# ShreenathKR2000/DFU-Multimodal

Hardware: AMD Instinct MI355X
Metric: images/sec (fusion fwd+bwd, bs=64/GPU) (higher is better)
Workload: dtype fwd ResNet50 bf16x3, ViT-B/16 Blocks fp16 (fp32 accumulate, residual stream, statistics); bwd bf16 MFMA; fp32 master weights / AdamW

## Files before the change

### dfu-multimodal_amd/csrc/gemm.hip

```cpp
#include <math.h>
#include <stdlib.h>

#include <type_traits>

#include "gemm_table.h"

using namespace dfu;

namespace {

inline int round8(int x) { return (x + 7) & ~7; }
inline int cdiv(int a, int b) { return (a + b - 1) / b; }

constexpr int kCUs = 256;
struct TileInfo {
  int tm, tn, occ;
  bool phased, tail_ok;
  double step_us, round_us;
  const Entry* kernels;
  const int* nkernels;
  int slots() const { return kCUs * occ; }
  int tiles(int M, int N) const { return cdiv(M, tm) * cdiv(N, tn); }
};
#define X(name, tm, tn, occ, phased, tail_ok, step_us, round_us) \
// ... 297 lines not shown
      DFU_CHECK_ARG(d->conv_k % BK == 0, "dfu_gemm: conv dgrad needs Kout %% 64 == 0");
      DFU_CHECK_ARG(d->K == d->conv_r * d->conv_s * d->conv_k, "dfu_gemm: conv dgrad K != RSK");
      DFU_CHECK_ARG(d->M == d->conv_n * d->conv_h * d->conv_w, "dfu_gemm: conv dgrad M != NHW");
      DFU_CHECK_ARG(d->conv_c % 8 == 0, "dfu_gemm: conv dgrad needs C %% 8 == 0");
      DFU_CHECK_ARG(d->b_mode == DFU_OPND_CONV_DGRAD_W, "dfu_gemm: conv dgrad needs DGRAD_W B");
    }
    if (d->b_mode == DFU_OPND_CONV_WGRAD_X) {
      DFU_CHECK_ARG(d->conv_c % 8 == 0, "dfu_gemm: conv wgrad needs C %% 8 == 0");
      DFU_CHECK_ARG(d->N == d->conv_r * d->conv_s * d->conv_c, "dfu_gemm: conv wgrad N != RSC");
      DFU_CHECK_ARG(d->K == d->conv_n * d->conv_p * d->conv_q, "dfu_gemm: conv wgrad K != NPQ");
    }
  }
  return DFU_OK;
}

}

extern "C" int dfu_gemm_stats_tiles(int32_t M) { return (M + 127) / 128; }

extern "C" int64_t dfu_gemm_workspace_bytes(const dfu_gemm_desc* d) {
  if (!d) return 0;
  const Plan pl = plan_gemm(d);
  if (!pl.entry) return 0;
  if (d->epilogue != DFU_EPI_F32_ACC) {
    if (!g_tail_split) return 0;
    if (d->a_mode == DFU_OPND_CONV_DGRAD && d->conv_stride > 1) {
      int64_t b = 0;
      for (const TileInfo& ti : kTiles) {
        const int64_t bt = ti.tail_ok ? (int64_t)ti.slots() * ti.tm * ti.tn * 4 : 0;
        if (bt > b) b = bt;
      }
      return b;
    }
    return tail_plan(d, pl).bytes;
  }
  return pl.split > 1 ? (int64_t)pl.split * d->M * d->N * 4 : 0;
}

extern "C" int dfu_gemm_plan(const dfu_gemm_desc* d, int32_t* tile, int32_t* split_k) {
  DFU_CHECK_ARG(d != nullptr && tile != nullptr && split_k != nullptr, "dfu_gemm_plan: null");
  Plan pl;
  const int rc = check_desc(d, false, &pl);
  if (rc != DFU_OK) return rc;
  *tile = pl.tile + 1;
  *split_k = pl.split;
  return DFU_OK;
}

extern "C" int dfu_gemm_set_persistent(int32_t mode) {
  const int old = (g_persistent ? 1 : 0) | (g_persistent_ps ? 2 : 0);
  g_persistent = (mode & 1) != 0;
  g_persistent_ps = (mode & 2) != 0;
  return old;
}

extern "C" int dfu_gemm_set_tail_split(int32_t enable) {
  const int old = g_tail_split;
  g_tail_split = enable != 0;
  return old;
}

extern "C" int dfu_gemm_set_inkernel_reduce(int32_t enable) {
  const int old = g_inkernel_reduce;
  g_inkernel_reduce = enable != 0;
  return old;
}

namespace {

struct Phase {
  int ph, pw, r0, s0, nr, ns, qh, qw, Hs, Ws;
};

Phase make_phase(const dfu_gemm_desc* d, int ph, int pw) {
  const int st = d->conv_stride, pad = d->conv_pad;
  Phase f;
  f.ph = ph;
  f.pw = pw;
  f.r0 = (ph + pad) % st;
  f.s0 = (pw + pad) % st;
  f.nr = f.r0 < d->conv_r ? (d->conv_r - f.r0 + st - 1) / st : 0;
  f.ns = f.s0 < d->conv_s ? (d->conv_s - f.s0 + st - 1) / st : 0;
  f.qh = (ph + pad - f.r0) / st;
  f.qw = (pw + pad - f.s0) / st;
  f.Hs = ph < d->conv_h ? (d->conv_h - ph + st - 1) / st : 0;
  f.Ws = pw < d->conv_w ? (d->conv_w - pw + st - 1) / st : 0;
  return f;
}

__global__ void k_phase_fill(bf16_t* __restrict__ C, int64_t ldc, const bf16_t* __restrict__ aux,
                             int64_t ldaux, int B, int Hs, int Ws, int H, int W, int st, int ph,
                             int pw, int N) {
  const int64_t rows = (int64_t)B * Hs * Ws;
  const int nv = N / 8;
  for (int64_t i = blockIdx.x * (int64_t)blockDim.x + threadIdx.x; i < rows * nv;
       i += (int64_t)gridDim.x * blockDim.x) {
    const int64_t m = i / nv;
    const int c = (int)(i - m * nv) * 8;
    const int b = (int)(m / ((int64_t)Hs * Ws));
    const int rem = (int)(m - (int64_t)b * Hs * Ws);
    const int h = rem / Ws, w = rem - (rem / Ws) * Ws;
    const int64_t row = ((int64_t)b * H + h * st + ph) * W + w * st + pw;
    const u32x4 v = aux ? *(const u32x4*)(aux + row * ldaux + c) : (u32x4){0u, 0u, 0u, 0u};
    *(u32x4*)(C + row * ldc + c) = v;
  }
}

int launch(const dfu_gemm_desc* d, const Plan& pl, const Phase* ph, hipStream_t s);

}

extern "C" int dfu_gemm(const dfu_gemm_desc* d, void* stream) {
  DFU_CHECK_ARG(d != nullptr, "dfu_gemm: null descriptor");
  Plan pl;
  const int rc = check_desc(d, true, &pl);
  if (rc != DFU_OK) return rc;
  hipStream_t s = (hipStream_t)stream;
  if (d->a_mode != DFU_OPND_CONV_DGRAD || d->conv_stride == 1) return launch(d, pl, nullptr, s);

  const int st = d->conv_stride;
  for (int ph = 0; ph < st; ++ph)
    for (int pw = 0; pw < st; ++pw) {
      const Phase f = make_phase(d, ph, pw);
      if (f.Hs == 0 || f.Ws == 0) continue;
      if (f.nr == 0 || f.ns == 0) {
        DFU_CHECK_ARG(d->epilogue == DFU_EPI_BF16 || d->epilogue == DFU_EPI_BF16_ADD,
                      "dfu_gemm: strided dgrad supports the BF16 / BF16_ADD epilogues");
        if (d->epilogue == DFU_EPI_BF16_ADD && d->aux == d->C && d->ldaux == d->ldc) continue;
        const int64_t n = (int64_t)d->conv_n * f.Hs * f.Ws * (d->N / 8);
        const int blocks = (int)((n + 255) / 256 < 4096 ? (n + 255) / 256 : 4096);
        hipLaunchKernelGGL(k_phase_fill, dim3(blocks), dim3(256), 0, s, (bf16_t*)d->C, d->ldc,
                           d->epilogue == DFU_EPI_BF16_ADD ? (const bf16_t*)d->aux : nullptr,
                           d->ldaux, d->conv_n, f.Hs, f.Ws, d->conv_h, d->conv_w, st, ph, pw,
                           d->N);
        DFU_LAUNCH_CHECK();
        continue;
      }
      dfu_gemm_desc pd = *d;
      pd.M = d->conv_n * f.Hs * f.Ws;
      pd.K = f.nr * f.ns * d->conv_k;
      const Plan pp = plan_gemm(&pd);
      if (!pp.entry) {
        dfu_set_error("dfu_gemm: no kernel for a dgrad phase");
        return DFU_E_UNSUPPORTED;
      }
      const int rc = launch(&pd, pp, &f, s);
      if (rc != DFU_OK) return rc;
    }
  return DFU_OK;
}

namespace {

inline bool is_ps(int tile) { return tile == T256x256ps || tile == T192x256ps; }

void fill_args(const dfu_gemm_desc* d, const Plan& pl, const Phase* ph, GemmArgs& a) {
  const TileInfo& ti = kTiles[pl.tile];
  a.M = d->M; a.N = d->N; a.K = d->K;
  a.ktiles = cdiv(d->K, BK);
  a.kt_per_split = cdiv(a.ktiles, pl.split);
  a.split = cdiv(a.ktiles, a.kt_per_split);
  a.tiles_m = cdiv(d->M, ti.tm);
  a.tiles_n = cdiv(d->N, ti.tn);
  a.A = (const bf16_t*)d->A; a.lda = d->lda;
  a.B = (const bf16_t*)d->B; a.ldb = d->ldb;
  a.C = d->C; a.ldc = d->ldc;
  a.alpha = d->alpha;
  a.bias = d->bias;
  a.aux = d->aux; a.ldaux = d->ldaux;
  a.aux_out = d->aux_out; a.ldaux_out = d->ldaux_out;
  a.stats = d->stats;
  a.n4 = (d->N % 4 == 0 && d->ldc % 4 == 0 && (d->aux == nullptr || d->ldaux % 4 == 0) &&
          (d->aux_out == nullptr || d->ldaux_out % 4 == 0))
             ? 1
             : 0;
  a.n8 = (a.n4 && d->N % 8 == 0 && d->ldc % 8 == 0 && ((uintptr_t)d->C & 15) == 0 &&
          (d->aux_out == nullptr || (d->ldaux_out % 8 == 0 && ((uintptr_t)d->aux_out & 15) == 0)))
             ? 1
             : 0;
  a.slab = nullptr;
  if (d->epilogue == DFU_EPI_F32_ACC && a.split > 1 && d->workspace != nullptr &&
      d->workspace_bytes >= (int64_t)a.split * d->M * d->N * 4)
    a.slab = (float*)d->workspace;
  a.counters = nullptr;
  if (a.slab != nullptr && g_inkernel_reduce && a.split <= 8 && d->tile_counters != nullptr &&
      d->tile_counters_len >= a.tiles_m * a.tiles_n && !ti.phased)
    a.counters = d->tile_counters;
  a.ep_tokens = d->ep_tokens;
  a.cn = d->conv_n; a.ch = d->conv_h; a.cw = d->conv_w; a.cc = d->conv_c;
  a.ck = d->conv_k; a.cr = d->conv_r; a.cs = d->conv_s;
  a.cstride = d->conv_stride; a.cpad = d->conv_pad; a.cp = d->conv_p; a.cq = d->conv_q;
  a.cpad_w = d->conv_pad;
  a.a_seg = d->a_seg;
  a.a_pix = d->a_seg ? d->a_seg : d->conv_c;
  a.a_lo_delta = d->a_seg ? ((const bf16_t*)d->a_lo - (const bf16_t*)d->A) : 0;
  a.ph_st = a.ph_h = a.ph_w = a.ph_r0 = a.ph_s0 = a.ph_H = a.ph_W = a.ph_S = 0;
  if (ph) {
    a.ch = ph->Hs; a.cw = ph->Ws; a.cr = ph->nr; a.cs = ph->ns;
    a.cstride = 1; a.cpad = ph->qh; a.cpad_w = ph->qw;
    a.ph_st = d->conv_stride; a.ph_h = ph->ph; a.ph_w = ph->pw;
    a.ph_r0 = ph->r0; a.ph_s0 = ph->s0;
    a.ph_H = d->conv_h; a.ph_W = d->conv_w; a.ph_S = d->conv_s;
  }
  static const int dbg = getenv("DFU_GEMM_DEBUG") ? atoi(getenv("DFU_GEMM_DEBUG")) : 0;
  a.dbg = dbg;
  a.m_ld_bound = round8(d->M);
  a.n_ld_bound = round8(d->N);
  if (d->a_mode >= DFU_OPND_CONV_FWD || d->b_mode >= DFU_OPND_CONV_FWD) {
    a.div_pq = make_fastdiv(a.cp * a.cq);
    a.div_q = make_fastdiv(a.cq);
    a.div_hw = make_fastdiv(a.ch * a.cw);
    a.div_w = make_fastdiv(a.cw);
    a.div_c = make_fastdiv(a.cc);
    a.div_k = make_fastdiv(a.ck);
    a.div_s = make_fastdiv(a.cs);
    if (d->b_mode == DFU_OPND_CONV_WGRAD_X) a.n_ld_bound = d->N;
  }
}

int check_ranges(const dfu_gemm_desc* d, const Plan& pl, const Phase* ph, GemmArgs& a) {
  const int64_t ea = d->a_mode == DFU_OPND_MNMAJOR ? (int64_t)(d->K - 1) * d->lda + round8(d->M)
                                                   : (int64_t)(d->M - 1) * d->lda + d->K;
  const int64_t eb = d->b_mode == DFU_OPND_MNMAJOR ? (int64_t)(d->K - 1) * d->ldb + round8(d->N)
                                                   : (int64_t)(d->N - 1) * d->ldb + d->K;
  if (is_ps(pl.tile))
    DFU_CHECK_ARG(2 * ea < kRsrcBytes && 2 * eb < kRsrcBytes,
                  "dfu_gemm: operands over 2 GiB need another tile than the buffer-DMA 256x256");
  a.a_bytes = (int)(2 * ea < kRsrcBytes ? 2 * ea : kRsrcBytes);
  a.b_bytes = (int)(2 * eb < kRsrcBytes ? 2 * eb : kRsrcBytes);
  const bool c32 = d->epilogue == DFU_EPI_F32 || d->epilogue == DFU_EPI_F32_RESID ||
                   d->epilogue == DFU_EPI_F32_ACC || d->epilogue == DFU_EPI_PATCH ||
                   d->epilogue == DFU_EPI_F32_STATS;
  int64_t c_rows = d->M;
  if (ph) c_rows = (int64_t)d->conv_n * d->conv_h * d->conv_w;
  if (d->epilogue == DFU_EPI_PATCH && d->ep_tokens > 0)
    c_rows = (int64_t)(d->M / d->ep_tokens) * (d->ep_tokens + 1);
  DFU_CHECK_ARG(c_rows * d->ldc * (c32 ? 4 : 2) < kRsrcBytes &&
                    (a.slab == nullptr || (int64_t)a.split * d->M * d->N * 4 < kRsrcBytes),
                "dfu_gemm: output larger than the 2 GiB epilogue buffer range");
  return DFU_OK;
}

int schedule(const dfu_gemm_desc* d, const Plan& pl, GemmArgs& a) {
  a.tail_full = a.tail_r = a.tail_s = a.tail_kps = 0;
  a.tslab = nullptr;
  const Tail t = tail_plan(d, pl);
  if (t.r > 0 && d->workspace != nullptr && d->workspace_bytes >= t.bytes &&
      d->tile_counters != nullptr && d->tile_counters_len >= t.r) {
    a.tail_full = t.full; a.tail_r = t.r; a.tail_s = t.s; a.tail_kps = t.kps;
    a.tslab = (float*)d->workspace;
    a.counters = d->tile_counters;
  }
  const int units = a.tail_r ? a.tail_full + a.tail_r * a.tail_s : a.tiles_m * a.tiles_n * a.split;
  const bool atomics = d->epilogue == DFU_EPI_F32_ACC && a.split > 1 && a.slab == nullptr;
  const bool pers = is_ps(pl.tile) ? g_persistent_ps : g_persistent;
  const int slots = kTiles[pl.tile].slots();
  return (pers && !atomics && units > slots) ? slots : units;
}

int reduce_slabs(const dfu_gemm_desc* d, const GemmArgs& a, hipStream_t s) {
  const int splits = a.split;
  const int64_t n = (int64_t)d->M * d->N;
  const bool vec = d->N % 4 == 0 && d->ldc % 4 == 0 && ((uintptr_t)d->C & 15) == 0;
  int64_t blocks = (vec ? n / 4 : n) / 256 + 1;
  if (blocks > 8192) blocks = 8192;
  if (blocks < kCUs && splits >= 8 && g_wide_reduce) {
    const int nw = splits < 16 ? splits : 16;
    const int64_t units = vec ? n / 4 : n;
    const unsigned wb = (unsigned)((units + 63) / 64);
    if (vec)
      hipLaunchKernelGGL(k_splitk_reduce_wide<true>, dim3(wb), dim3(64 * nw), 0, s, a.slab,
                         splits, d->M, d->N, (float*)d->C, d->ldc);
    else
      hipLaunchKernelGGL(k_splitk_reduce_wide<false>, dim3(wb), dim3(64 * nw), 0, s, a.slab,
                         splits, d->M, d->N, (float*)d->C, d->ldc);
  } else if (vec)
    hipLaunchKernelGGL(k_splitk_reduce, dim3((unsigned)blocks), dim3(256), 0, s, a.slab, splits,
                       d->M, d->N, (float*)d->C, d->ldc);
  else
    hipLaunchKernelGGL(k_splitk_reduce_scalar,
                       dim3((unsigned)((d->N + 255) / 256), (unsigned)(d->M < 4096 ? d->M : 4096)),
                       dim3(256), 0, s, a.slab, splits, d->M, d->N, (float*)d->C, d->ldc);
  DFU_LAUNCH_CHECK();
  return DFU_OK;
}

int launch(const dfu_gemm_desc* d, const Plan& pl, const Phase* ph, hipStream_t s) {
  GemmArgs a;
  fill_args(d, pl, ph, a);
  DFU_CHECK_ARG(!(kTiles[pl.tile].phased && d->epilogue == DFU_EPI_F32_ACC && a.split > 1 &&
                  a.slab == nullptr),
                "dfu_gemm: split-K on the phased 256x256 tile needs a workspace "
                "(dfu_gemm_workspace_bytes)");
  const int rc = check_ranges(d, pl, ph, a);
  if (rc != DFU_OK) return rc;
  const int nwg = schedule(d, pl, a);
  hipLaunchKernelGGL(pl.entry->fn, dim3(nwg), dim3(pl.entry->threads), 0, s, a);
  DFU_LAUNCH_CHECK();
  if (a.slab != nullptr && a.counters == nullptr) return reduce_slabs(d, a, s);
  return DFU_OK;
}

}
```

### dfu-multimodal_amd/csrc/gemm_kernel.h

```cpp
#pragma once
#include "common.h"

namespace dfu {

constexpr int BK = 64;
constexpr int LDS_MAX = 160 * 1024;

template <int TM_, int TN_, int OCC_ = 1, int NST_ = 0, int NW_ = 8>
struct Tile {
  static constexpr int TM = TM_, TN = TN_, OCC = OCC_, NW = NW_, NT = 64 * NW_;
  static constexpr int WGM = NW == 4 ? 2 : (TM == 256 && TN == 128) ? 4 : 2;
  static constexpr int WGN = NW / WGM;
  static constexpr int WTM = TM / WGM, WTN = TN / WGN;
  static constexpr int FM = WTM / 16, FN = WTN / 16;
  static constexpr int NLDA = TM / (8 * NW), NLDB = TN / (8 * NW);
  static constexpr int A_BYTES = TM * BK * 2, B_BYTES = TN * BK * 2;
  static constexpr int STAGE_BYTES = A_BYTES + B_BYTES;
  static constexpr int STATS_BYTES = WGM * TN * 3 * 4;
  static constexpr int NSTAGE =
      NST_ ? NST_ : ((OCC == 1 && 3 * STAGE_BYTES + STATS_BYTES <= LDS_MAX) ? 3 : 2);
  static constexpr int LDS_BYTES = NSTAGE * STAGE_BYTES;
  static constexpr int DMA_PER_STAGE = NLDA + NLDB;
  static_assert(OCC * (LDS_BYTES + STATS_BYTES) <= LDS_MAX, "LDS for the requested occupancy");
};
// ... 533 lines not shown
  for (int i = 0; i < T::FM; ++i)
#pragma unroll
    for (int j = 0; j < T::FN; ++j)
      __builtin_amdgcn_raw_buffer_store_b128(__builtin_bit_cast(u32x4, acc[i][j]), rs,
                                             off(s, i * T::FN + j), 0, 16);
  int* flag = (int*)red;
  asm volatile("s_waitcnt vmcnt(0)" ::: "memory");
  __builtin_amdgcn_s_barrier();
  if (tid == 0) {
    const int old = __hip_atomic_fetch_add(p.counters + r, 1, __ATOMIC_RELAXED,
                                           __HIP_MEMORY_SCOPE_AGENT);
    const int last = old == S - 1;
    if (last) __hip_atomic_store(p.counters + r, 0, __ATOMIC_RELAXED, __HIP_MEMORY_SCOPE_AGENT);
    *flag = last;
  }
  asm volatile("s_waitcnt vmcnt(0) lgkmcnt(0)" ::: "memory");
  __builtin_amdgcn_s_barrier();
  if (!*flag) return false;
  for (int k = 0; k < S; k += 2) {
    const int k1 = k + 1 < S ? k + 1 : k;
    f32x4 x0[T::FM][T::FN], x1[T::FM][T::FN];
#pragma unroll
    for (int i = 0; i < T::FM; ++i)
#pragma unroll
      for (int j = 0; j < T::FN; ++j) {
        x0[i][j] = __builtin_bit_cast(
            f32x4, __builtin_amdgcn_raw_buffer_load_b128(rs, off(k, i * T::FN + j), 0, 16));
        x1[i][j] = __builtin_bit_cast(
            f32x4, __builtin_amdgcn_raw_buffer_load_b128(rs, off(k1, i * T::FN + j), 0, 16));
      }
#pragma unroll
    for (int i = 0; i < T::FM; ++i)
#pragma unroll
      for (int j = 0; j < T::FN; ++j) {
        f32x4 a = k == 0 ? x0[i][j] : acc[i][j] + x0[i][j];
        if (k1 != k) a = a + x1[i][j];
        acc[i][j] = a;
      }
  }
  return true;
}

template <int EPI, class T>
constexpr bool aux_prefetch() {
  return (EPI == DFU_EPI_BF16_DGELU || EPI == DFU_EPI_BF16_ADD) && T::FM * T::FN <= 16;
}
template <class T>
struct AuxPre {
  u32x2 v[T::FM][T::FN];
};

DFU_DEV int64_t out_row(const GemmArgs& p, int m);

template <int AMODE, int EPI, class T>
DFU_DEV void aux_load(const GemmArgs& p, int m0, int n0, int tid, AuxPre<T>& pre) {
  const int lane = tid & 63, wave = tid >> 6;
  const int wr = wave / T::WGN, wc = wave % T::WGN;
  const int lrow = lane & 15, lcol = 4 * (lane >> 4);
  const rsrc_t ra = make_rsrc(p.aux);
  const bool n4 = p.n4 != 0;
#pragma unroll
  for (int i = 0; i < T::FM; ++i) {
    const int m = m0 + wr * T::WTM + 16 * i + lrow;
    const bool okm = m < p.M;
    const int mc = okm ? m : 0;
    const int64_t mo = AMODE == DFU_OPND_CONV_DGRAD ? out_row(p, mc) : (int64_t)mc;
#pragma unroll
    for (int j = 0; j < T::FN; ++j) {
      const int n = n0 + wc * T::WTN + 16 * j + lcol;
      const int64_t e = mo * p.ldaux + n;
      if (n4) {
        pre.v[i][j] = __builtin_amdgcn_raw_buffer_load_b64(ra, boff(okm && n < p.N, e * 2), 0, 0);
      } else {
        uint32_t h[4];
#pragma unroll
        for (int q = 0; q < 4; ++q)
          h[q] = __builtin_amdgcn_raw_buffer_load_b16(ra, boff(okm && n + q < p.N, (e + q) * 2), 0, 0);
        pre.v[i][j] = (u32x2){h[0] | (h[1] << 16), h[2] | (h[3] << 16)};
      }
    }
  }
}
DFU_DEV void unpack4(u32x2 x, float* v) {
  v[0] = lo_bf(x[0]);
  v[1] = hi_bf(x[0]);
  v[2] = lo_bf(x[1]);
  v[3] = hi_bf(x[1]);
}

template <int AMODE, int EPI, class T>
DFU_DEV void epilogue(const GemmArgs& p, f32x4 (&acc)[T::FM][T::FN], int m0, int n0, int sidx,
                      float* red, int tid, const AuxPre<T>& pre) {
  constexpr bool kPre = aux_prefetch<EPI, T>();
  constexpr int FM = T::FM, FN = T::FN, WTM = T::WTM, WTN = T::WTN, WGM = T::WGM;
  constexpr int TM = T::TM, TN = T::TN;
  const int lane = tid & 63, wave = tid >> 6;
  const int wr = wave / T::WGN, wc = wave % T::WGN;
  const int lrow = lane & 15, lcol = 4 * (lane >> 4);
  const bool n4 = p.n4 != 0;
  const int M = p.M, N = p.N;
  const rsrc_t rc = make_rsrc(p.C);

  if constexpr (EPI == DFU_EPI_BF16_STATS || EPI == DFU_EPI_F32_STATS) {
    float cnt = 0.f;
#pragma unroll
    for (int i = 0; i < FM; ++i) cnt += (m0 + wr * WTM + 16 * i + lrow < M) ? 1.f : 0.f;
    cnt = row16_sum(cnt);
#pragma unroll
    for (int j = 0; j < FN; ++j) {
#pragma unroll
      for (int r = 0; r < 4; ++r) {
        float s = 0.f;
#pragma unroll
        for (int i = 0; i < FM; ++i) {
          const int m = m0 + wr * WTM + 16 * i + lrow;
          const float v = EPI == DFU_EPI_BF16_STATS ? bf2f(f2bf(acc[i][j][r] * p.alpha))
                                                    : acc[i][j][r] * p.alpha;
          acc[i][j][r] = v;
          s += (m < M) ? v : 0.f;
        }
        s = row16_sum(s);
        const float mean = cnt > 0.f ? s / cnt : 0.f;
        float q = 0.f;
#pragma unroll
        for (int i = 0; i < FM; ++i) {
          const int m = m0 + wr * WTM + 16 * i + lrow;
          const float d = acc[i][j][r] - mean;
          q += (m < M) ? d * d : 0.f;
        }
        q = row16_sum(q);
        if (lrow == 0) {
          const int c = wc * WTN + 16 * j + lcol + r;
          red[(wr * TN + c) * 3 + 0] = s;
          red[(wr * TN + c) * 3 + 1] = q;
          red[(wr * TN + c) * 3 + 2] = cnt;
        }
      }
    }
    asm volatile("s_waitcnt lgkmcnt(0)" ::: "memory");
    __builtin_amdgcn_s_barrier();
    const rsrc_t rs = make_rsrc(p.stats);
    constexpr int HALVES = TM / 128;
    for (int idx = tid; idx < TN * HALVES; idx += T::NT) {
      const int c = idx % TN, h = idx / TN;
      const int n = n0 + c;
      float S = 0.f, Q = 0.f, Cn = 0.f;
#pragma unroll
      for (int w = 0; w < WGM; ++w) {
        if ((w * WTM) / 128 != h) continue;
        const float s1 = red[(w * TN + c) * 3 + 0], q1 = red[(w * TN + c) * 3 + 1];
        const float c1 = red[(w * TN + c) * 3 + 2];
        if (c1 <= 0.f) continue;
        if (Cn > 0.f) {
          const float d = s1 / c1 - S / Cn;
          Q += q1 + d * d * Cn * c1 / (Cn + c1);
        } else {
          Q = q1;
        }
        S += s1;
        Cn += c1;
      }
      const bool ok = n < N && m0 + 128 * h < M;
      const int64_t blk = m0 / 128 + h;
      __builtin_amdgcn_raw_buffer_store_b32(__float_as_uint(S), rs,
                                            boff(ok, ((blk * 2 + 0) * N + n) * 4), 0, 0);
      __builtin_amdgcn_raw_buffer_store_b32(__float_as_uint(Q), rs,
                                            boff(ok, ((blk * 2 + 1) * N + n) * 4), 0, 0);
    }
#pragma unroll
    for (int i = 0; i < FM; ++i) {
      const int m = m0 + wr * WTM + 16 * i + lrow;
      float v[FN][4];
#pragma unroll
      for (int j = 0; j < FN; ++j)
#pragma unroll
        for (int r = 0; r < 4; ++r) v[j][r] = acc[i][j][r];
      if constexpr (EPI == DFU_EPI_BF16_STATS) {
        st_row_bf16<FN>(rc, (int64_t)m * p.ldc, m < M, n0 + wc * WTN, N, p.n8, n4, lane, v);
      } else if (p.aux_out) {
        float lo[FN][4];
#pragma unroll
        for (int j = 0; j < FN; ++j)
#pragma unroll
          for (int r = 0; r < 4; ++r) {
            const float h = bf2f(f2bf(v[j][r]));
            lo[j][r] = v[j][r] - h;
            v[j][r] = h;
          }
        st_row_bf16<FN>(rc, (int64_t)m * p.ldc, m < M, n0 + wc * WTN, N, p.n8, n4, lane, v);
        st_row_bf16<FN>(make_rsrc(p.aux_out), (int64_t)m * p.ldaux_out, m < M, n0 + wc * WTN, N,
                        p.n8, n4, lane, lo);
      } else {
#pragma unroll
        for (int j = 0; j < FN; ++j) {
          const int n = n0 + wc * WTN + 16 * j + lcol;
          st4_f32(rc, (int64_t)(m < M ? m : 0) * p.ldc + n, m < M, n, N, n4, v[j]);
        }
      }
    }
  } else {
    constexpr bool kBias = EPI == DFU_EPI_BF16 || EPI == DFU_EPI_BF16_RELU || EPI == DFU_EPI_F32 ||
                           EPI == DFU_EPI_F32_RESID || EPI == DFU_EPI_BF16_GELU ||
                           EPI == DFU_EPI_PATCH;
    float bias[FN][4];
#pragma unroll
    for (int j = 0; j < FN; ++j)
#pragma unroll
      for (int r = 0; r < 4; ++r) bias[j][r] = 0.f;
    if (kBias && p.bias) load_bias<FN>(p.bias, n0 + wc * WTN, N, lane, bias);
    const rsrc_t ra = make_rsrc(p.aux);
    const rsrc_t ro = make_rsrc(EPI == DFU_EPI_F32_ACC ? (const void*)p.slab : p.aux_out);
#pragma unroll
    for (int i = 0; i < FM; ++i) {
      const int m = m0 + wr * WTM + 16 * i + lrow;
      const bool okm = m < M;
      const int mc = okm ? m : 0;
      const int64_t mo = AMODE == DFU_OPND_CONV_DGRAD ? out_row(p, mc) : (int64_t)mc;
      const int n0w = n0 + wc * WTN;
      float v[FN][4];
#pragma unroll
      for (int j = 0; j < FN; ++j)
#pragma unroll
        for (int r = 0; r < 4; ++r) v[j][r] = acc[i][j][r] * p.alpha + bias[j][r];
      if constexpr (EPI == DFU_EPI_BF16 || EPI == DFU_EPI_BF16_RELU) {
        if constexpr (EPI == DFU_EPI_BF16_RELU) {
#pragma unroll
          for (int j = 0; j < FN; ++j)
#pragma unroll
            for (int r = 0; r < 4; ++r) v[j][r] = fmaxf(v[j][r], 0.f);
        }
        st_row_bf16<FN>(rc, mo * p.ldc, okm, n0w, N, p.n8, n4, lane, v);
      } else if constexpr (EPI == DFU_EPI_BF16_GELU) {
        float g[FN][4], d[FN][4];
#pragma unroll
        for (int j = 0; j < FN; ++j)
#pragma unroll
          for (int r = 0; r < 4; ++r) gelu_and_grad(v[j][r], g[j][r], d[j][r]);
        st_row_bf16<FN>(ro, mo * p.ldaux_out, okm, n0w, N, p.n8, n4, lane, d);
        st_row_bf16<FN>(rc, mo * p.ldc, okm, n0w, N, p.n8, n4, lane, g);
      } else if constexpr (EPI == DFU_EPI_BF16_DGELU || EPI == DFU_EPI_BF16_ADD) {
#pragma unroll
        for (int j = 0; j < FN; ++j) {
          const int n = n0w + 16 * j + lcol;
          float x[4];
          if constexpr (kPre)
            unpack4(pre.v[i][j], x);
          else
            ld4_bf16(ra, mo * p.ldaux + n, okm, n, N, n4, x);
#pragma unroll
          for (int r = 0; r < 4; ++r)
            v[j][r] = (EPI == DFU_EPI_BF16_DGELU) ? v[j][r] * x[r] : v[j][r] + x[r];
        }
        st_row_bf16<FN>(rc, mo * p.ldc, okm, n0w, N, p.n8, n4, lane, v);
      } else {
#pragma unroll
        for (int j = 0; j < FN; ++j) {
          const int n = n0w + 16 * j + lcol;
          if constexpr (EPI == DFU_EPI_F32) {
            st4_f32(rc, mo * p.ldc + n, okm, n, N, n4, v[j]);
          } else if constexpr (EPI == DFU_EPI_F32_RESID) {
            float x[4];
            ld4_f32(ra, mo * p.ldaux + n, okm, n, N, n4, x);
#pragma unroll
            for (int r = 0; r < 4; ++r) v[j][r] += x[r];
            st4_f32(rc, mo * p.ldc + n, okm, n, N, n4, v[j]);
          } else if constexpr (EPI == DFU_EPI_F32_ACC) {
            if (p.slab != nullptr) {
              if (p.counters != nullptr)
                st4_f32<16>(ro, ((int64_t)sidx * M + mc) * N + n, okm, n, N, n4, v[j]);
              else
                st4_f32(ro, ((int64_t)sidx * M + mc) * N + n, okm, n, N, n4, v[j]);
            } else if (p.split > 1) {
              float* C = (float*)p.C + (int64_t)mc * p.ldc + n;
              for (int r = 0; r < 4; ++r)
                if (okm && n + r < N) atomicAdd(C + r, v[j][r]);
            } else {
              float c[4];
              ld4_f32(rc, (int64_t)mc * p.ldc + n, okm, n, N, n4, c);
#pragma unroll
              for (int r = 0; r < 4; ++r) v[j][r] += c[r];
              st4_f32(rc, (int64_t)mc * p.ldc + n, okm, n, N, n4, v[j]);
            }
          } else if constexpr (EPI == DFU_EPI_PATCH) {
            const int Tt = p.ep_tokens;
            const int b = mc / Tt, t = mc - b * Tt;
            float pe[4];
            ld4_f32(ra, (int64_t)(1 + t) * p.ldaux + n, okm, n, N, n4, pe);
#pragma unroll
            for (int r = 0; r < 4; ++r) v[j][r] += pe[r];
            st4_f32(rc, ((int64_t)b * (Tt + 1) + 1 + t) * p.ldc + n, okm, n, N, n4, v[j]);
          }
        }
      }
    }
    if constexpr (EPI == DFU_EPI_F32_ACC) {
      if (p.slab != nullptr && p.counters != nullptr) splitk_finish<T>(p, m0, n0, red, tid);
    }
  }
}

template <int AMODE, int BMODE, int EPI, int TM, int TN, int OCC = 1, int NST = 0, int NW = 8,
          bool X3 = false>
__global__ __launch_bounds__(64 * NW, OCC) void gemm_kernel(const GemmArgs p) {
  using T = Tile<TM, TN, OCC, NST, NW>;
  constexpr int WGN = T::WGN, WTM = T::WTM, WTN = T::WTN;
  constexpr int FM = T::FM, FN = T::FN, NSTAGE = T::NSTAGE;
  constexpr int SCRATCH = (EPI == DFU_EPI_BF16_STATS || EPI == DFU_EPI_F32_STATS)
                              ? T::STATS_BYTES
                              : 16;
  __shared__ __attribute__((aligned(16))) char smem[T::LDS_BYTES + SCRATCH];
  const int tid = threadIdx.x;
  const int lane = tid & 63;
  const int wave = tid >> 6;
  const int wr = wave / WGN, wc = wave % WGN;

  constexpr bool kTail = NW == 8 && FM * FN <= 8 && EPI != DFU_EPI_F32_ACC;
  const int tiles = p.tiles_m * p.tiles_n;
  const int units = kTail && p.tail_r ? p.tail_full + p.tail_r * p.tail_s : tiles * p.split;
  const int nwg = gridDim.x;
  const int bid = blockIdx.x;
  int wg = bid;
  if (nwg >= 16) {
    const int xcd = bid & 7, q = nwg >> 3, r = nwg & 7;
    wg = (xcd < r ? xcd * (q + 1) : r * (q + 1) + (xcd - r) * q) + (bid >> 3);
  }
  const int full = units / nwg;
  const int rounds = full + (bid < units - full * nwg ? 1 : 0);
  if (rounds == 0) return;
  auto unit_at = [&](int i) { return i * nwg + (i < full ? wg : bid); };

  auto unit_geom = [&](int u, int& m0, int& n0, int& kb, int& nk) {
    constexpr int GROUP_M = 4;
    int s, t, kps;
    if (kTail && p.tail_r && u >= p.tail_full) {
      const int v = u - p.tail_full;
      s = v / p.tail_r;
      t = p.tail_full + (v - s * p.tail_r);
      kps = p.tail_kps;
    } else {
      s = u / tiles;
      t = u - s * tiles;
      kps = p.kt_per_split;
    }
    const int band = GROUP_M * p.tiles_n;
    const int g0 = (t / band) * GROUP_M;
    const int gm = min(GROUP_M, p.tiles_m - g0);
    const int within = t - (t / band) * band;
    m0 = (g0 + within % gm) * TM;
    n0 = (within / gm) * TN;
    kb = s * kps;
    nk = min(p.ktiles, kb + kps) - kb;
  };
  int total = 0;
  for (int i = 0; i < rounds; ++i) {
    int m0_, n0_, kb_, nk_;
    unit_geom(unit_at(i), m0_, n0_, kb_, nk_);
    total += nk_;
  }

  LoadState<T::NLDA> sa;
  LoadState<T::NLDB> sb;
  int iu = 0, ik = 0, im0, in0, ikb, ink;
  unit_geom(unit_at(0), im0, in0, ikb, ink);
  load_init<AMODE, T::NLDA, NW>(p, sa, p.A, p.lda, im0, p.M, tid);
  load_init<BMODE, T::NLDB, NW>(p, sb, p.B, p.ldb, in0, p.N, tid);
  auto issue_next = [&](char* stage) {
    if (!(p.dbg & 4)) {
    issue_tile<AMODE, T::NLDA, NW, true, X3>(p, sa, p.A, p.lda, p.m_ld_bound, ikb + ik, p.K, tid,
                                         stage);
    issue_tile<BMODE, T::NLDB, NW>(p, sb, p.B, p.ldb, p.n_ld_bound, ikb + ik, p.K, tid,
                               stage + T::A_BYTES);
    }
    if (++ik == ink) {
      ik = 0;
      if (++iu < rounds) {
        unit_geom(unit_at(iu), im0, in0, ikb, ink);
        load_init<AMODE, T::NLDA, NW>(p, sa, p.A, p.lda, im0, p.M, tid);
        load_init<BMODE, T::NLDB, NW>(p, sb, p.B, p.ldb, in0, p.N, tid);
      }
    }
  };

  f32x4 acc[FM][FN];
#pragma unroll
  for (int i = 0; i < FM; ++i)
#pragma unroll
    for (int j = 0; j < FN; ++j) acc[i][j] = (f32x4){0.f, 0.f, 0.f, 0.f};

  constexpr bool AK = kcontig<AMODE>();
  constexpr bool BKc = kcontig<BMODE>();
  auto compute = [&](const char* la) {
    const char* lb = la + T::A_BYTES;
    static_assert(!X3 || (FM * FN < 32 && AK && BKc),
                  "interleaved pairs: K-contiguous operands, at most 64x64 per wave");
    if constexpr (FM * FN >= 32) {
#pragma unroll
      for (int ks = 0; ks < 2; ++ks) {
        bf16x8 fa[FM], fb[FN];
#pragma unroll
        for (int i = 0; i < FM; ++i) fa[i] = read_frag<AK>(la, wr * WTM + i * 16, ks, lane);
#pragma unroll
        for (int j = 0; j < FN; ++j) fb[j] = read_frag<BKc>(lb, wc * WTN + j * 16, ks, lane);
        if constexpr (!AK || !BKc) {
          lds_reads_retired();
#pragma unroll
          for (int i = 0; i < FM; ++i) pin(fa[i]);
#pragma unroll
          for (int j = 0; j < FN; ++j) pin(fb[j]);
        }
#pragma unroll
        for (int i = 0; i < FM; ++i)
#pragma unroll
          for (int j = 0; j < FN; ++j)
            acc[i][j] = __builtin_amdgcn_mfma_f32_16x16x32_bf16(fb[j], fa[i], acc[i][j], 0, 0, 0);
      }
    } else {
      bf16x8 fa[2][FM], fb[2][FN];
#pragma unroll
      for (int ks = 0; ks < 2; ++ks) {
#pragma unroll
        for (int i = 0; i < FM; ++i) fa[ks][i] = read_frag<AK>(la, wr * WTM + i * 16, ks, lane);
#pragma unroll
        for (int j = 0; j < FN; ++j) fb[ks][j] = read_frag<BKc>(lb, wc * WTN + j * 16, ks, lane);
      }
      __builtin_amdgcn_sched_barrier(0);
      if constexpr (!AK || !BKc) {
        lds_reads_retired();
#pragma unroll
        for (int ks = 0; ks < 2; ++ks) {
#pragma unroll
          for (int i = 0; i < FM; ++i) pin(fa[ks][i]);
#pragma unroll
          for (int j = 0; j < FN; ++j) pin(fb[ks][j]);
        }
      }
      if constexpr (X3) {
#pragma unroll
        for (int t = 0; t < 3; ++t)
#pragma unroll
          for (int i = 0; i < FM; ++i)
#pragma unroll
            for (int j = 0; j < FN; ++j)
              acc[i][j] = __builtin_amdgcn_mfma_f32_16x16x32_bf16(fb[t == 2][j], fa[t == 1][i],
                                                                 acc[i][j], 0, 0, 0);
      } else {
#pragma unroll
        for (int ks = 0; ks < 2; ++ks)
#pragma unroll
          for (int i = 0; i < FM; ++i)
#pragma unroll
            for (int j = 0; j < FN; ++j)
              acc[i][j] =
                  __builtin_amdgcn_mfma_f32_16x16x32_bf16(fb[ks][j], fa[ks][i], acc[i][j], 0, 0, 0);
      }
    }
  };

  const int E = (p.dbg & 1) ? 0 : epi_stores<EPI, T>(p);
  AuxPre<T> pre;
  float* red = (float*)(smem + T::LDS_BYTES);
  unsigned hist = 0;
  int ci = 0, cu = unit_at(0), ck = 0, cm0, cn0, ckb, cnk;
  unit_geom(cu, cm0, cn0, ckb, cnk);
#pragma unroll
  for (int s = 0; s < NSTAGE - 1; ++s)
    if (s < total) issue_next(smem + s * T::STAGE_BYTES);
  int slot = 0;
  for (int g = 0; g < total; ++g) {
    const int later = min(NSTAGE - 2, total - 1 - g);
    const unsigned win = hist & ((1u << (NSTAGE - 1)) - 1u);
    if (win == 0 && later == NSTAGE - 2)
      wait_vmcnt<T::DMA_PER_STAGE * (NSTAGE - 2)>();
    else
      wait_vm_le<63>(T::DMA_PER_STAGE * later + E * __builtin_popcount(win));
    __builtin_amdgcn_s_barrier();
    if (g + NSTAGE - 1 < total) {
      const int is = slot == 0 ? NSTAGE - 1 : slot - 1;
      issue_next(smem + is * T::STAGE_BYTES);
    }
    if constexpr (aux_prefetch<EPI, T>())
      if (ck + 1 == cnk) aux_load<AMODE, EPI, T>(p, cm0, cn0, tid, pre);
    if (!(p.dbg & 2)) compute(smem + slot * T::STAGE_BYTES);
    slot = slot == NSTAGE - 1 ? 0 : slot + 1;
    hist <<= 1;
    if (++ck == cnk) {
      bool epi = true;
      if constexpr (kTail)
        if (p.tail_r && cu >= p.tail_full) epi = tail_reduce<T>(p, acc, cu - p.tail_full, red, tid);
      if (epi && !(p.dbg & 1))
        epilogue<AMODE, EPI, T>(p, acc, cm0, cn0, cu / tiles, red, tid, pre);
#pragma unroll
      for (int i = 0; i < FM; ++i)
#pragma unroll
        for (int j = 0; j < FN; ++j) acc[i][j] = (f32x4){0.f, 0.f, 0.f, 0.f};
      hist |= 1u;
      ck = 0;
      if (++ci < rounds) {
        cu = unit_at(ci);
        unit_geom(cu, cm0, cn0, ckb, cnk);
      }
    }
  }
}

}
```

### dfu-multimodal_amd/csrc/gemm_table.h

```cpp
#pragma once
#ifdef __HIP__
#include "gemm_kernel.h"
#endif

#define DFU_TILES(X)                                                                   \
  X(128x128, 128, 128, 1, false, true, 0.57, 4.8)                                      \
  X(256x128, 256, 128, 1, false, false, 0.89, 8.3)                                     \
  X(128x256, 128, 256, 1, false, false, 0.90, 7.4)                                     \
  X(256x256, 256, 256, 1, false, false, 1.41, 13.9)                                    \
  X(128x128o2, 128, 128, 2, false, true, 0.70, 6.1)                                    \
  X(128x128w4, 128, 128, 2, false, false, 0.65, 6.1)                      \
  X(256x256p8, 256, 256, 1, true, false, 3.0, 20.0)     \
  X(256x256ps, 256, 256, 1, true, false, 3.0, 20.0)                    \
  X(192x256ps, 192, 256, 1, true, false, 3.0, 20.0)    \
  X(256x64, 256, 64, 1, false, false, 3.0, 20.0)          \
  X(128x64o2, 128, 64, 2, false, false, 3.0, 20.0)

namespace dfu {
struct GemmArgs;
typedef void (*gemm_fn)(const GemmArgs);
constexpr int kF16Key = 64;
constexpr int kX3Key = 128;
struct Entry {
  int a, b, e, tile;
  gemm_fn fn;
  int lds_bytes;
  int threads;
};
#define X(name, ...) T##name,
enum TileId { DFU_TILES(X) NTILES };
#undef X
#define X(name, ...)                   \
  extern const Entry kTable##name[]; \
  extern const int kTable##name##N;
DFU_TILES(X)
#undef X
}

#define DFU_ENTRY(A, B, E, TMv, TNv, TID)                                             \
  {                                                                                   \
    A, B, E, TID, &dfu::gemm_kernel<A, B, E, TMv, TNv>, dfu::Tile<TMv, TNv>::LDS_BYTES, \
        dfu::Tile<TMv, TNv>::NT                                                       \
  }
#define DFU_ENTRY_OCC(A, B, E, TMv, TNv, OCCv, TID)                       \
  {                                                                       \
    A, B, E, TID, &dfu::gemm_kernel<A, B, E, TMv, TNv, OCCv>,             \
        dfu::Tile<TMv, TNv, OCCv>::LDS_BYTES, dfu::Tile<TMv, TNv, OCCv>::NT   \
  }
#define DFU_ENTRY_NST(A, B, E, TMv, TNv, NSTv, TID)                       \
  {                                                                       \
    A, B, E, TID, &dfu::gemm_kernel<A, B, E, TMv, TNv, 1, NSTv>,          \
        dfu::Tile<TMv, TNv, 1, NSTv>::LDS_BYTES, dfu::Tile<TMv, TNv, 1, NSTv>::NT \
  }
#define DFU_ENTRY_W4(A, B, E, TMv, TNv, OCCv, TID)                              \
  {                                                                             \
    A, B, E, TID, &dfu::gemm_kernel<A, B, E, TMv, TNv, OCCv, 0, 4>,             \
        dfu::Tile<TMv, TNv, OCCv, 0, 4>::LDS_BYTES, dfu::Tile<TMv, TNv, OCCv, 0, 4>::NT \
  }
#define DFU_ENTRY_X3(A, B, E, TMv, TNv, OCCv, NWv, TID)                                      \
  {                                                                                          \
    A, B, (E) | dfu::kX3Key, TID, &dfu::gemm_kernel<A, B, E, TMv, TNv, OCCv, 0, NWv, true>,   \
        dfu::Tile<TMv, TNv, OCCv, 0, NWv>::LDS_BYTES, dfu::Tile<TMv, TNv, OCCv, 0, NWv>::NT  \
  }
```

### dfu-multimodal_amd/dfu_hip/_lib.py

```python
import ctypes
import os
import re

_HERE = os.path.dirname(os.path.abspath(__file__))
LIB_PATH = os.environ.get("DFU_HIP_LIB") or os.path.join(_HERE, "libdfu_hip.so")
HEADER_PATH = os.path.normpath(os.path.join(_HERE, "..", "..", "include", "dfu_hip.h"))

c_int32 = ctypes.c_int32
c_int64 = ctypes.c_int64
c_float = ctypes.c_float
c_uint64 = ctypes.c_uint64
c_void_p = ctypes.c_void_p
c_char_p = ctypes.c_char_p

OPND_KMAJOR, OPND_MNMAJOR, OPND_CONV_FWD, OPND_CONV_DGRAD, OPND_CONV_DGRAD_W, OPND_CONV_WGRAD_X = range(6)
(EPI_BF16, EPI_BF16_RELU, EPI_BF16_GELU, EPI_F32, EPI_F32_RESID, EPI_BF16_DGELU, EPI_BF16_ADD,
 EPI_F32_ACC, EPI_F32_ACC_CONVW, EPI_BF16_STATS, EPI_PATCH, EPI_F32_STATS,
 EPI_BF16_DSTATS, EPI_X3_GELU, EPI_F16_DUAL, EPI_F16_GELU) = range(16)
OPERAND_BF16, OPERAND_F16 = 0, 1

DFU_E_INVALID = 1001
DFU_E_UNSUPPORTED = 1002


class GemmDesc(ctypes.Structure):
    _fields_ = [
        ("M", c_int32), ("N", c_int32), ("K", c_int32),
        ("a_mode", c_int32), ("b_mode", c_int32),
        ("A", c_void_p), ("lda", c_int64),
        ("B", c_void_p), ("ldb", c_int64),
        ("C", c_void_p), ("ldc", c_int64),
        ("epilogue", c_int32), ("alpha", c_float),
        ("bias", c_void_p),
        ("aux", c_void_p), ("ldaux", c_int64),
        ("aux_out", c_void_p), ("ldaux_out", c_int64),
        ("stats", c_void_p),
        ("split_k", c_int32),
        ("ep_tokens", c_int32),
        ("conv_n", c_int32), ("conv_h", c_int32), ("conv_w", c_int32), ("conv_c", c_int32),
        ("conv_k", c_int32), ("conv_r", c_int32), ("conv_s", c_int32),
        ("conv_stride", c_int32), ("conv_pad", c_int32),
        ("conv_p", c_int32), ("conv_q", c_int32),
        ("tile", c_int32),
        ("workspace", c_void_p), ("workspace_bytes", c_int64),
        ("tile_counters", c_void_p), ("tile_counters_len", c_int32),
        ("operand_type", c_int32),
        ("a_seg", c_int32), ("a_lo", c_void_p),
        ("x3_pairs", c_int32),
    ]


class ReduceEntry(ctypes.Structure):
    _fields_ = [("partial", c_void_p), ("stride", c_int64), ("out", c_void_p),
                ("blocks", c_int32), ("D", c_int32)]


REDUCE_BATCH = 8
P = c_void_p
I32 = c_int32
I64 = c_int64
F = c_float

PROTOTYPES = {
    "dfu_last_error_string": [],
    "dfu_version": [],
    "dfu_zero": [P, I64, P],
    "dfu_streams_abort_capture": [P, I32, P],
    "dfu_stream_capture_status": [P, P],
    "dfu_stream_create": [I32, P],
    "dfu_stream_destroy": [P],
    "dfu_stream_wait": [P, P],
    "dfu_gemm": [ctypes.POINTER(GemmDesc), P],
    "dfu_gemm_stats_tiles": [I32],
    "dfu_gemm_workspace_bytes": [ctypes.POINTER(GemmDesc)],
    "dfu_gemm_plan": [ctypes.POINTER(GemmDesc), ctypes.POINTER(c_int32), ctypes.POINTER(c_int32)],
    "dfu_gemm_set_persistent": [I32],
    "dfu_gemm_set_inkernel_reduce": [I32],
    "dfu_gemm_set_tail_split": [I32],
    "dfu_gemm_f32": [I32, I32, I32, P, I64, I64, P, I64, I64, P, I64, P, I32, I32, P, I64, P],
    "dfu_gemm_f32_workspace_bytes": [I32, I32, I32],
    "dfu_pack_conv_weight": [P, P, I32, I32, I32, I32, P],
    "dfu_conv_grad_krsc_to_oihw": [P, P, I32, I32, I32, I32, P],
    "dfu_cast_rows_bf16": [P, I64, P, I64, I32, I32, P],
    "dfu_transpose_bf16": [P, I32, I32, P],
    "dfu_cast_rows_f32": [P, I64, P, I64, I32, I32, P],
    "dfu_cast_rows_f16": [P, I64, P, I64, I32, I32, P],
    "dfu_im2col_f32": [P, I64, I64, I64, I64, I32, I32, I32, I32, I32, I32, I32, I32, I32, I32, P, I32, P],
    "dfu_patchify_f32": [P, I64, I64, I64, I64, I32, I32, I32, I32, I32, P, P],
    "dfu_col2im_f32": [P, I32, I32, I32, I32, I32, I32, I32, I32, I32, I32, I32, P, P],
    "dfu_unpatchify_f32": [P, I32, I32, I32, I32, I32, P, P],
    "dfu_gradcam": [P, I32, I64, I64, I64, P, I32, I64, I64, I64, I32, I32, I32, P, P],
    "dfu_saliency": [P, I32, I32, I32, P, P],
    "dfu_bn_finalize": [P, I32, I32, I32, P, P, F, F, P, P, P, P, P, P, P, P, P, I32, P],
    "dfu_bn_finalize_ws_bytes": [I32, I32],
    "dfu_bn_bwd_finalize_ws_bytes": [I32, I32],
    "dfu_bn_eval_coeffs": [P, P, P, P, F, I32, P, P, P],
    "dfu_bn_apply": [P, P, P, P, I32, P, I64, I32, P],
    "dfu_bn_tile_stats": [P, I64, I32, P, P],
    "dfu_bn_apply_mask": [P, P, P, P, I32, P, P, I64, I32, P],
    "dfu_bn_bwd_blocks": [I64, I32],
    "dfu_bn_bwd_reduce": [P, P, P, I32, P, P, P, P, I64, I32, P, P],
    "dfu_bn_bwd_finalize": [P, I32, I64, I32, P, P, I32, P, P, P, P, P, I32, P],
    "dfu_bn_bwd_apply": [P, P, P, I32, P, P, P, P, P, I64, I32, P, P, P],
    "dfu_bn_bwd_ws_bytes": [I64, I32],
    "dfu_bn_bwd": [P, P, P, I32, P, P, P, P, P, I64, I32, I32, P, P, P, P, P, I64, P, I32, P],
    "dfu_maxpool_fwd": [P, I32, I32, I32, I32, P, P, I32, I32, P],
    "dfu_maxpool_bn_fwd": [P, P, P, I32, I32, I32, I32, P, P, I32, I32, P],
    "dfu_maxpool_bwd": [P, P, I32, I32, I32, I32, I32, I32, P, P],
    "dfu_avgpool_fwd": [P, I32, I32, I32, P, P],
    "dfu_avgpool_bwd": [P, I32, I32, I32, P, P],
    "dfu_layernorm_fwd": [P, I64, I32, I32, P, P, F, P, I64, I32, P, P, P],
    "dfu_ln_bwd_blocks": [I32],
    "dfu_layernorm_bwd": [P, I64, I32, P, I64, P, P, P, I32, I32, P, I64, P, P, P, P],
    "dfu_reduce_partials": [P, I32, I32, I32, P, P, P],
    "dfu_reduce_partials_batch": [ctypes.POINTER(ReduceEntry), I32, P],
    "dfu_attention_fwd": [P, I32, I32, I32, I32, F, P, P, P],
    "dfu_attention_fwd_f16": [P, I32, I32, I32, I32, F, P, P, P, P],
    "dfu_attention_bwd": [P, P, P, P, I32, I32, I32, I32, F, P, P, P],
    "dfu_attention_bwd_qkv16": [P, P, P, P, I32, I32, I32, I32, F, P, P, P],
    "dfu_attention_npad": [I32],
    "dfu_vit_cls_rows": [P, P, P, I32, I32, I32, P],
    "dfu_vit_embed_bwd": [P, I32, I32, I32, P, P, P, P, P, P],
    "dfu_colsum": [P, I32, I64, I32, I32, P, P, P],
    "dfu_colsum_blocks": [I32],
    "dfu_gather_rows_f32": [P, I64, I32, I32, I32, I32, P, I64, P],
    "dfu_scatter_rows_f32": [P, I64, I32, I32, I32, I32, P, I64, P],
    "dfu_relu_fwd": [P, P, I64, I32, P],
    "dfu_relu_bwd": [P, P, P, I64, I32, P],
    "dfu_dropout_fwd": [P, P, P, I64, F, c_uint64, P, I32, P],
    "dfu_dropout_bwd": [P, P, P, I64, F, I32, P],
    "dfu_concat2_bf16": [P, I32, I32, P, I32, I32, I32, P, P],
    "dfu_split2_f32": [P, I32, I32, I32, I32, P, P, P],
    "dfu_ce_weighted_fwd": [P, P, P, I32, I32, P, P, P],
    "dfu_ce_weighted_bwd": [P, P, I32, I32, P, P],
    "dfu_adamw": [P, P, P, P, P, I32, P, I32, F, F, F, F, F, P, P],
    "dfu_adamw_flat": [P, P, P, P, I64, F, F, F, F, F, P, P, P, P, I64, I64, P],
    "dfu_step_increment": [P, P],
    "dfu_argmax_rows": [P, I32, I32, P, P],
    "dfu_softmax_rows": [P, I32, I32, P, P],
    "dfu_metrics_accumulate": [P, P, I32, I32, P, P, P, P, P],
    "dfu_split_x3": [P, I64, I32, I32, I32, P, I32, P, I64, P],
    "dfu_pack_conv_weight_x3": [P, P, I32, I32, I32, I32, I32, P],
    "dfu_stem_conv_x3": [P, I64, I64, I64, I64, I32, I32, I32, I32, P, I32, I32, I32, I32, I32,
                         P, P, P, P, P],
    "dfu_stem_wgrad_ws_bytes": [I32, I32, I32],
    "dfu_stem_wgrad_x3": [P, I64, I64, I64, I64, I32, I32, I32, I32, P, I32, I32, I32, I32, I32,
                          P, P, I64, P],
    "dfu_maxpool_bn_fwd_x3": [P, P, P, P, I32, I32, I32, I32, P, P, P, P, I32, I32, P],
    "dfu_im2col_f32_x3": [P, I64, I64, I64, I64, I32, I32, I32, I32, I32, I32, I32, I32, I32, I32, P, P, I32, P],
    "dfu_patchify_f32_x3": [P, I64, I64, I64, I64, I32, I32, I32, I32, I32, P, P],
    "dfu_bn_apply_x3": [P, P, P, P, P, P, I32, I32, P, P, P, P, P, I64, I32, P],
    "dfu_maxpool_fwd_x3": [P, I32, I32, I32, I32, P, P, P, I32, I32, P],
    "dfu_avgpool_fwd_x3": [P, P, I32, I32, I32, P, P],
    "dfu_layernorm_fwd_x3": [P, I64, I32, I32, P, P, F, P, P, P, P, P],
    "dfu_layernorm_fwd_h16": [P, I64, I32, I32, P, P, F, P, P, P, P, P],
    "dfu_gelu_x3": [P, I64, I32, P, P, P, P],
    "dfu_attention_fwd_f32": [P, I32, I32, I32, I32, F, I32, P, P, P, P, P],
    "dfu_resize_ksize": [I32, I32],
    "dfu_resize_coeffs": [I32, I32, P, P],
    "dfu_resize_batch": [P, P, P, I32, I32, I32, P, P, P],
    "dfu_augment_normalize": [P, P, I32, I32, I32, P, P, P, P, P],
    "dfu_augment_views": [P, I32, P, P, I32, I32, I32, I32, P, P, P, P, P],
    "dfu_tta_reduce": [P, I32, I32, I32, P, P, P],
    "dfu_binary_eval_counts": [P, P, P, I32, P, P],
}
_RESTYPE = {"dfu_last_error_string": c_char_p, "dfu_gemm_workspace_bytes": c_int64,
            "dfu_gemm_f32_workspace_bytes": c_int64, "dfu_bn_finalize_ws_bytes": c_int64,
            "dfu_bn_bwd_finalize_ws_bytes": c_int64, "dfu_stem_wgrad_ws_bytes": c_int64,
            "dfu_bn_bwd_ws_bytes": c_int64}


def header_symbols(path=HEADER_PATH):
    with open(path) as f:
        text = f.read()
    return sorted(set(re.findall(r"^\s*(?:int|int64_t|const char\*)\s+(dfu_\w+)\s*\(", text, re.M)))


class DfuError(RuntimeError):
    def __init__(self, msg, code=0):
        super().__init__(msg)
        self.code = code


_lib = None


def load():
    global _lib
    if _lib is not None:
        return _lib
    if not os.path.exists(LIB_PATH):
        raise DfuError(
            f"libdfu_hip.so not found at {LIB_PATH}; build it with "
            f"`make -C dfu-multimodal_amd` (or __graft_entry__.build()). There is no fallback.")
    lib = ctypes.CDLL(LIB_PATH)
    for name, argtypes in PROTOTYPES.items():
        fn = getattr(lib, name)
        fn.argtypes = argtypes
        fn.restype = _RESTYPE.get(name, c_int32)
    _lib = lib
    return lib


def check(rc, what=""):
    if rc != 0:
        msg = load().dfu_last_error_string()
        msg = msg.decode() if msg else ""
        raise DfuError(f"{what or 'dfu call'} failed (rc={rc}): {msg}", rc)
```

### dfu-multimodal_amd/dfu_hip/functional.py

```python
import math
import os
import weakref

import torch

from . import _lib as L
from . import ops
from .streams import (current_stream, join_grad_streams, new_stream, on_stream,
                      side_stream, stream_wait, wgrad_stream)
from .streams import grad_streams as _grad_streams

BF16 = torch.bfloat16
F32 = torch.float32

PRECISIONS = ("bf16", "bf16x3", "mixed", "parity")
STAGE_MODES = ("bf16", "bf16x3", "fp16")
DEFAULT_PRECISION = "parity"
_precision = [DEFAULT_PRECISION]


def set_precision(mode):
    if mode not in PRECISIONS:
        raise ValueError(f"precision must be one of {PRECISIONS}, got {mode!r}")
    old = _precision[0]
# ... 128 lines not shown
    def __enter__(self):
        _concurrent_encoders[0] += 1

    def __exit__(self, *exc):
        _concurrent_encoders[0] -= 1


class _Beside:

    def __init__(self, stream):
        self.ws = stream
        self.cur = current_stream() if stream is not None else None

    def run(self, fn, *tensors):
        if self.ws is None:
            return fn()
        stream_wait(self.ws, self.cur)
        with on_stream(self.ws):
            for t in tensors:
                t.record_stream(self.ws)
            return fn()


def grads_done(*params):
    if not _grad_ready_hooks:
        return
    hooks = tuple(_grad_ready_hooks)
    for p in params:
        if p is not None:
            for h in hooks:
                h(p)


def module_param(mod, name):
    p = mod._parameters
    if name in p:
        return p[name]
    b = mod._buffers
    return b[name] if name in b else getattr(mod, name)


def wants(p):
    return p is not None and p.requires_grad


def _empty(shape, dtype, device):
    return torch.empty(shape, dtype=dtype, device=device)


def nhwc_bf16(x):
    if x.dtype != BF16:
        x = x.to(BF16)
    if not x.is_contiguous(memory_format=torch.channels_last):
        x = x.contiguous(memory_format=torch.channels_last)
    return x


def rows_view(x):
    B, C, H, W = x.shape
    return x.permute(0, 2, 3, 1).reshape(B * H * W, C)


def from_rows(r, B, H, W, C):
    return r.view(B, H, W, C).permute(0, 3, 1, 2)


def krsc_strided(w):
    return (w.dim() == 4 and not w.is_contiguous()
            and w.is_contiguous(memory_format=torch.channels_last))


def _rows2d(w):
    if krsc_strided(w):
        return w.permute(0, 2, 3, 1).reshape(w.shape[0], -1)
    return w.reshape(w.shape[0], -1)


def weight_bf16_rows(w, ld=None):
    w2 = _rows2d(w.detach())
    sh = getattr(w, "_dfu_shadow", None)
    if sh is not None and (ld is None or ld == w2.shape[1]):
        if w._version != getattr(w, "_dfu_shadow_version", -1):
            ops.cast_rows_bf16(w2, out=sh)
            w._dfu_shadow_version = w._version
            w._dfu_sgen = getattr(w, "_dfu_sgen", 0) - 1
        return sh
    return ops.cast_rows_bf16(w2, ld_out=ld)


def weight_f16_rows(w):
    flat = getattr(w, "_dfu_flat", None)
    if flat is not None and flat.shadow is not None:
        if flat.shadow16 is None:
            flat.enable_f16()
        sh = w._dfu_shadow16
        if w._version != getattr(w, "_dfu_shadow16_version", -1):
            ops.cast_rows_f16(_rows2d(w.detach()), out=sh)
            w._dfu_shadow16_version = w._version
        return sh
    return ops.cast_rows_f16(_rows2d(w.detach()))


def weight_bf16_T(w):
    sh = weight_bf16_rows(w)
    flat = getattr(w, "_dfu_flat", None)
    if flat is None or sh is not getattr(w, "_dfu_shadow", None):
        return None
    if getattr(w, "_dfu_shadow_T", None) is None:
        flat.add_transposed(w)
        w._dfu_tgen = None
    if w._dfu_tgen != getattr(w, "_dfu_sgen", 0):
        ops.transpose_bf16(sh, out=w._dfu_shadow_T)
        w._dfu_tgen = getattr(w, "_dfu_sgen", 0)
    return w._dfu_shadow_T


_DGRAD_FLIP = os.environ.get("DFU_DGRAD_FLIP", "1") != "0"


def conv_weight_flipped(w):
    if not _DGRAD_FLIP or not krsc_strided(w):
        return None
    sh = weight_bf16_rows(w)
    flat = getattr(w, "_dfu_flat", None)
    if flat is None or sh is not getattr(w, "_dfu_shadow", None):
        return None
    if getattr(w, "_dfu_shadow_F", None) is None:
        flat.add_flipped(w)
    key = (flat.gen, getattr(w, "_dfu_shadow_version", None))
    if w._dfu_fkey != key:
        w._dfu_flip_jobs.launch()
        w._dfu_fkey = key
    return w._dfu_shadow_F


_DGRAD_T1X1_MAXC = int(os.environ.get("DFU_DGRAD_T1X1_MAXC", "64"))


def conv1x1_weight_T(conv, geom):
    if (geom.r == 1 and geom.s == 1 and geom.stride == 1 and geom.pad == 0
            and geom.c <= _DGRAD_T1X1_MAXC):
        return weight_bf16_T(conv.weight)
    return None


def conv_weight_bf16(w):
    if (w.shape[2] == 1 and w.shape[3] == 1) or krsc_strided(w):
        return weight_bf16_rows(w)
    return ops.pack_conv_weight(w.detach())


def weight_x3_rows(w, seg=None):
    return ops.split_x3(w.detach().reshape(w.shape[0], -1), ops.X3_B, seg=seg)


_X3_PAIRS = os.environ.get("DFU_X3_PAIRS", "1") != "0"


def conv_weight_x3(w):
    flat = getattr(w, "_dfu_flat", None)
    if _X3_PAIRS and flat is not None:
        from .optim import x3_pair_weight
        if x3_pair_weight(w):
            if flat.shadow_x3 is None:
                flat.enable_x3()
            sh = w._dfu_shadow_x3
            if w._version != getattr(w, "_dfu_shadow_x3_version", -1):
                src = w.detach().permute(0, 2, 3, 1).reshape(-1, 32)
                ops.split_x3_into(src.contiguous(), ops.X3_PAIRS, sh.view(-1, 64))
                w._dfu_shadow_x3_version = w._version
            return sh
    if _X3_PAIRS:
        if w.shape[2] == 1 and w.shape[3] == 1:
            return ops.split_x3(w.detach().reshape(w.shape[0], -1), ops.X3_PAIRS)
        return ops.pack_conv_weight_x3(w.detach(), ops.X3_PAIRS)
    if w.shape[2] == 1 and w.shape[3] == 1:
        return weight_x3_rows(w)
    return ops.pack_conv_weight_x3(w.detach())


def _take_x3(x):
    hi = rows_view(nhwc_bf16(x.detach()))
    lo = getattr(x, "_dfu_lo", None)
    if lo is not None:
        try:
            del x._dfu_lo
        except AttributeError:
            pass
        return hi, lo
    return hi, torch.zeros_like(hi)


class BNState:

    def __init__(self, bn, M, C, device):
        self.bn = bn
        self.M, self.C = M, C
        self.training = bn.training or not bn.track_running_stats
        self.coef4 = _empty((4, C), F32, device)
        self.scale, self.shift, self.mean, self.invstd = self.coef4.unbind(0)

    def forward_coeffs(self, stats):
        bn = self.bn
        if self.training:
            track = bn.track_running_stats and bn.training
            mom = bn.momentum if bn.momentum is not None else 0.1
            mp = module_param
            ops.bn_finalize(stats, self.M, self.C, mp(bn, "weight"), mp(bn, "bias"), bn.eps, mom,
                            mp(bn, "running_mean") if track else None,
                            mp(bn, "running_var") if track else None,
                            mp(bn, "num_batches_tracked") if track else None,
                            self.mean, self.invstd, self.scale, self.shift)
        else:
            ops.bn_eval_coeffs(bn.weight, bn.bias, bn.running_mean, bn.running_var, bn.eps,
                               self.scale, self.shift)
            self.mean.copy_(bn.running_mean)
            ops.bn_eval_coeffs(None, None, bn.running_mean, bn.running_var, bn.eps,
                               self.invstd, _empty((self.C,), F32, self.mean.device))

    def backward(self, dout, y, out, relu, dy, dres):
        bn = self.bn
        w, b = module_param(bn, "weight"), module_param(bn, "bias")
        dgamma = grad_buffer(w) if wants(w) else None
        dbeta = grad_buffer(b) if wants(b) else None
        ops.bn_bwd(dout, y, out, relu, self.mean, self.invstd, w, self.M, self.C, dy,
                   dres, dgamma, dbeta, batch_stats=self.training, scale=self.scale,
                   shift=self.shift)
        grads_done(w, b)


def conv_fwd(x_rows, geom, w_krsc, y, stats):
    g = geom
    M = g.n * g.p * g.q
    if g.r == 1 and g.s == 1 and g.stride == 1 and g.pad == 0:
        ops.gemm(M, g.k, g.c, x_rows, g.c, w_krsc, g.c, y, g.k, epilogue=L.EPI_BF16_STATS,
                 stats=stats)
    else:
        K = g.r * g.s * g.c
        ops.gemm(M, g.k, K, x_rows, 0, w_krsc, K, y, g.k, a_mode=L.OPND_CONV_FWD,
                 epilogue=L.EPI_BF16_STATS, stats=stats, conv=g)


def conv_fwd_x3(x_pair, geom, w3, y, stats, y_lo=None):
    g = geom
    hi, lo = x_pair
    M = g.n * g.p * g.q
    pairs = _X3_PAIRS
    C3 = (2 if pairs else 3) * g.c
    K3 = g.r * g.s * C3
    xk = dict(x3=True, a_lo=lo, x3_pairs=pairs)
    out = dict(aux_out=y_lo, ldaux_out=g.k if y_lo is not None else 0)
    if g.r == 1 and g.s == 1 and g.stride == 1 and g.pad == 0:
        ops.gemm(M, g.k, C3, hi, g.c, w3, C3, y, g.k, epilogue=L.EPI_F32_STATS, stats=stats,
                 **xk, **out)
    else:
        g3 = ops.ConvGeom(g.n, g.h, g.w, C3, g.k, g.r, g.s, g.stride, g.pad)
        ops.gemm(M, g.k, K3, hi, 0, w3, K3, y, g.k, a_mode=L.OPND_CONV_FWD,
                 epilogue=L.EPI_F32_STATS, stats=stats, conv=g3, **xk, **out)


def conv_dgrad(dy_rows, geom, w_krsc, dx, add=None, w_flip=None, w_t=None):
    g = geom
    Mx = g.n * g.h * g.w
    if w_t is not None and g.r == 1 and g.s == 1 and g.stride == 1 and g.pad == 0:
        ops.gemm(Mx, g.c, g.k, dy_rows, g.k, w_t, g.k, dx, g.c,
                 epilogue=L.EPI_BF16_ADD if add is not None else L.EPI_BF16, aux=add,
                 ldaux=g.c if add is not None else 0)
        return
    if w_flip is not None and add is None and g.stride == 1:
        gd = ops.ConvGeom(g.n, g.p, g.q, g.k, g.c, g.r, g.s, 1, g.r - 1 - g.pad)
        if (gd.p, gd.q) == (g.h, g.w) and g.r - 1 - g.pad >= 0:
            K = g.r * g.s * g.k
            ops.gemm(Mx, g.c, K, dy_rows, 0, w_flip, K, dx, g.c, a_mode=L.OPND_CONV_FWD,
                     epilogue=L.EPI_BF16, conv=gd)
            return
    epi = L.EPI_BF16_ADD if add is not None else L.EPI_BF16
    aux, ld_aux = add, (g.c if add is not None else 0)
    if g.r == 1 and g.s == 1 and g.stride == 1 and g.pad == 0:
        ops.gemm(Mx, g.c, g.k, dy_rows, g.k, w_krsc, g.c, dx, g.c, b_mode=L.OPND_MNMAJOR,
                 epilogue=epi, aux=aux, ldaux=ld_aux)
    else:
        ops.gemm(Mx, g.c, g.r * g.s * g.k, dy_rows, 0, w_krsc, g.r * g.s * g.c, dx, g.c,
                 a_mode=L.OPND_CONV_DGRAD, b_mode=L.OPND_CONV_DGRAD_W, epilogue=epi, aux=aux,
                 ldaux=ld_aux, conv=g)


def conv_wgrad(dy_rows, x_rows, geom, dw):
    g = geom
    M = g.n * g.p * g.q
    if g.r == 1 and g.s == 1 and g.stride == 1 and g.pad == 0:
        ops.gemm(g.k, g.c, M, dy_rows, g.k, x_rows, g.c, dw, g.c, a_mode=L.OPND_MNMAJOR,
                 b_mode=L.OPND_MNMAJOR, epilogue=L.EPI_F32_ACC)
    elif krsc_strided(dw):
        N = g.r * g.s * g.c
        ops.gemm(g.k, N, M, dy_rows, g.k, x_rows, 0, _rows2d(dw), N, a_mode=L.OPND_MNMAJOR,
                 b_mode=L.OPND_CONV_WGRAD_X, epilogue=L.EPI_F32_ACC, conv=g)
    else:
        N = g.r * g.s * g.c
        acc = _empty((g.k, N), F32, dy_rows.device)
        ops.zero_(acc)
        ops.gemm(g.k, N, M, dy_rows, g.k, x_rows, 0, acc, N, a_mode=L.OPND_MNMAJOR,
                 b_mode=L.OPND_CONV_WGRAD_X, epilogue=L.EPI_F32_ACC, conv=g)
        ops.conv_grad_krsc_to_oihw(acc, dw)


def _geom(conv, B, H, W):
    Cout, Cin, R, S = conv.weight.shape
    return ops.ConvGeom(B, H, W, Cin, Cout, R, S, conv.stride[0], conv.padding[0])


_STEM_FUSED = os.environ.get("DFU_STEM_FUSED", "1") != "0"


class StemFn(torch.autograd.Function):

    KP = 160

    @staticmethod
    def forward(ctx, x, w, gamma, beta, mod):
        conv, bn = mod.conv1, mod.bn1
        B, C, H, W = x.shape
        R = S = conv.weight.shape[2]
        st, pad = conv.stride[0], conv.padding[0]
        Kp = ((C * R * S + 15) // 16) * 16
        xf = x.detach().float() if x.dtype != F32 else x.detach()
        wb = weight_bf16_rows(w, ld=Kp)
        Cout = w.shape[0]
        x3 = _x3(mod)
        fused = x3 and _STEM_FUSED and Kp == 160 and ops.stem_conv_x3_ok(xf, w, st, pad)
        if fused:
            y, y_lo, stats, col, P, Q = ops.stem_conv_x3(xf, w.detach(), st, pad, want_col=False)
        elif x3:
            (col, col_lo), P, Q = ops.im2col_f32_x3(xf, R, S, st, pad, Kp)
        else:
            col, P, Q = ops.im2col_f32(xf, R, S, st, pad, Kp)
        M = B * P * Q
        if not fused:
            y = _empty((M, Cout), BF16, x.device)
            stats = _empty((ops.stats_tiles(M), 2, Cout), F32, x.device)
        bns = BNState(bn, M, Cout, x.device)
        if x3:
            a = _empty((M * Cout // 8,), torch.uint8, x.device)
            if not fused:
                y_lo = _empty((M, Cout), BF16, x.device)
                if _X3_PAIRS and Kp % 32 == 0:
                    w3, K3, pairs = ops.split_x3(w.detach().reshape(Cout, -1), ops.X3_PAIRS,
                                                 seg=Kp), 2 * Kp, True
                else:
                    w3, K3, pairs = weight_x3_rows(w, seg=Kp), 3 * Kp, False
                ops.gemm(M, Cout, K3, col, Kp, w3, K3, y, Cout, epilogue=L.EPI_F32_STATS,
                         stats=stats, x3=True, a_lo=col_lo, x3_pairs=pairs, aux_out=y_lo,
                         ldaux_out=Cout)
                del col_lo
            bns.forward_coeffs(stats)
            out_lo, out, am, P2, Q2 = ops.maxpool_bn_fwd_x3(y, y_lo, bns.scale, bns.shift, B, P,
                                                            Q, Cout, relu_mask=a)
            del y_lo
        else:
            ops.gemm(M, Cout, Kp, col, Kp, wb, Kp, y, Cout, epilogue=L.EPI_BF16_STATS,
                     stats=stats)
            bns.forward_coeffs(stats)
            a = None
            out, am, P2, Q2 = ops.maxpool_fwd(y, B, P, Q, Cout, scale=bns.scale,
                                              shift=bns.shift)
        ctx.mod = mod
        ctx.bns = bns
        ctx.x3 = x3
        ctx.dims = (B, C, H, W, P, Q, P2, Q2, Cout, Kp, R, S, st, pad)
        ctx.x_requires_grad = x.requires_grad
        ctx.fused = fused
        ctx.save_for_backward(xf if fused else col, y, a, am, wb)
        res = out.permute(0, 3, 1, 2)
        if x3:
            res._dfu_lo = out_lo
        return res

    @staticmethod
    def backward(ctx, gout):
        col, y, a, am, wb = ctx.saved_tensors
        B, C, H, W, P, Q, P2, Q2, Cout, Kp, R, S, st, pad = ctx.dims
        mod = ctx.mod
        g = rows_view(nhwc_bf16(gout))
        da = ops.maxpool_bwd(g, am, B, P, Q, Cout, P2, Q2).view(B * P * Q, Cout)
        M = B * P * Q
        dy = torch.empty_like(y)
        if ctx.x3:
            ctx.bns.backward(da, y, a, 3, dy, None)
        else:
            ctx.bns.backward(da, y, None, 2, dy, None)
        w = mod.conv1.weight
        if wants(w):
            dw = grad_buffer(w).view(Cout, -1)
            K = C * R * S
            if ctx.fused:
                ops.stem_wgrad_x3(col, dy, dw, st, pad)
            else:
                ops.gemm(Cout, K, M, dy, Cout, col, col.stride(0), dw, K, a_mode=L.OPND_MNMAJOR,
                         b_mode=L.OPND_MNMAJOR, epilogue=L.EPI_F32_ACC)
            grads_done(w)
        dx = None
        if ctx.x_requires_grad:
            wkn = wb
            dcol = _empty((M, Kp), F32, y.device)
            ops.gemm(M, Kp, Cout, dy, Cout, wkn, Kp, dcol, Kp, b_mode=L.OPND_MNMAJOR,
                     epilogue=L.EPI_F32)
            dx = ops.col2im_f32(dcol, B, C, H, W, R, S, st, pad, P, Q, Kp)
        return dx, None, None, None, None


def _fire_grad_hooks(probe, grad):
    for hook in list((probe._backward_hooks or {}).values()):
        hook(grad)


class BottleneckFn(torch.autograd.Function):

    @staticmethod
    def forward(ctx, x, *params_and_mod):
        mod = params_and_mod[-1]
        mm = mod._modules
        x3mode = _x3(mod)
        xin3 = _take_x3(x) if x3mode else None
        x = nhwc_bf16(x.detach())
        B, Cin, H, W = x.shape
        dev = x.device
        xr = rows_view(x)
        g1 = _geom(mm["conv1"], B, H, W)
        g2 = _geom(mm["conv2"], B, g1.p, g1.q)
        g3 = _geom(mm["conv3"], B, g2.p, g2.q)
        w1 = conv_weight_bf16(mm["conv1"].weight)
        w2 = conv_weight_bf16(mm["conv2"].weight)
        w3 = conv_weight_bf16(mm["conv3"].weight)
        M1 = B * g1.p * g1.q
        M2 = B * g2.p * g2.q
        planes, outc = g1.k, g3.k

        def conv_bn(xrows, geom, w, bnmod, relu, residual=None, mask=None):
            M = geom.n * geom.p * geom.q
            y = _empty((M, geom.k), BF16, dev)
            stats = _empty((ops.stats_tiles(M), 2, geom.k), F32, dev)
            conv_fwd(xrows, geom, w, y, stats)
            st = BNState(bnmod, M, geom.k, dev)
            st.forward_coeffs(stats)
            out = _empty((M, geom.k), BF16, dev)
            ops.bn_apply(y, st.scale, st.shift, residual, relu, out, M, geom.k, mask=mask)
            return y, out, st

        def conv_bn_x3(xpair, geom, w3x, bnmod, relu, res=None, res_mode=0, want_pair=True,
                       want_f32=False):
            M = geom.n * geom.p * geom.q
            y = _empty((M, geom.k), BF16, dev)
            y_lo = _empty((M, geom.k), BF16, dev)
            stats = _empty((ops.stats_tiles(M), 2, geom.k), F32, dev)
            conv_fwd_x3(xpair, geom, w3x, y, stats, y_lo=y_lo)
            st = BNState(bnmod, M, geom.k, dev)
            st.forward_coeffs(stats)
            out = _empty((M, geom.k), BF16, dev) if want_pair else None
            lo = _empty((M, geom.k), BF16, dev) if want_pair else None
            of = _empty((M, geom.k), F32, dev) if want_f32 else None
            rhi, rlo = res if res_mode == 2 else (res, None)
            mask = _empty((M * geom.k // 8,), torch.uint8, dev) if relu else None
            ops.bn_apply_x3(y, st.scale, st.shift, rhi, res_mode, relu, M, geom.k, out_lo=lo,
                            out_bf16=out, out_f32=of, residual_lo=rlo, y_lo=y_lo, relu_mask=mask)
            return y, out, lo, of, st, mask

        out_lo = None
        masks = None
        if x3mode:
            y1, a1, a1_lo, _, s1, m1 = conv_bn_x3(xin3, g1, conv_weight_x3(mm["conv1"].weight),
                                                   mm["bn1"], True)
            y2, a2, a2_lo, _, s2, m2 = conv_bn_x3((a1, a1_lo), g2,
                                                   conv_weight_x3(mm["conv2"].weight), mm["bn2"],
                                                   True)
            masks = (m1, m2)
            del a1_lo
        else:
            y1, a1, s1 = conv_bn(xr, g1, w1, mm["bn1"], True)
            y2, a2, s2 = conv_bn(a1, g2, w2, mm["bn2"], True)
        if mm.get("downsample") is not None:
            dconv, dbn = mm.get("downsample")[0], mm.get("downsample")[1]
            gd = _geom(dconv, B, H, W)
            wd = conv_weight_bf16(dconv.weight)
            if x3mode:
                yd, _, _, idn, sd, _ = conv_bn_x3(xin3, gd, conv_weight_x3(dconv.weight), dbn,
                                                  False, want_pair=False, want_f32=True)
                res, res_mode = idn, 1
            else:
                yd, idn, sd = conv_bn(xr, gd, wd, dbn, False)
        else:
            gd = wd = yd = sd = None
            idn = xr
            res, res_mode = xin3, 2
        if x3mode:
            y3, out, out_lo, _, s3, mask3 = conv_bn_x3((a2, a2_lo), g3,
                                                        conv_weight_x3(mm["conv3"].weight),
                                                        mm["bn3"], True, res=res,
                                                        res_mode=res_mode)
            del a2_lo, res, xin3
        else:
            mask3 = _empty((M2 * outc // 8,), torch.uint8, dev)
            y3, out, s3 = conv_bn(a2, g3, w3, mm["bn3"], True, residual=idn, mask=mask3)
        ctx.x3 = x3mode
        ctx.mod = mod
        ctx.geo = (g1, g2, g3, gd)
        ctx.bns = (s1, s2, s3, sd)
        ctx.shape = (B, Cin, H, W)
        ctx.x_requires_grad = ctx.needs_input_grad[0]
        ctx.probes = None
        if getattr(mod, "_probe", False):
            ctx.probes = (from_rows(a1, B, g1.p, g1.q, planes).detach().requires_grad_(True),
                          from_rows(a2, B, g2.p, g2.q, planes).detach().requires_grad_(True))
            mod._probes = ctx.probes
        ctx.masks = masks
        ctx.save_for_backward(xr, y1, a1, y2, a2, y3, mask3, w1, w2,
                              w3, *( (yd, wd) if yd is not None else ()))
        res = from_rows(out, B, g3.p, g3.q, outc)
        if out_lo is not None:
            res._dfu_lo = out_lo
        return res

    @staticmethod
    def backward(ctx, gout):
        saved = ctx.saved_tensors
        xr, y1, a1, y2, a2, y3, out, w1, w2, w3 = saved[:10]
        yd, wd = (saved[10], saved[11]) if len(saved) > 10 else (None, None)
        mod = ctx.mod
        mm = mod._modules
        g1, g2, g3, gd = ctx.geo
        s1, s2, s3, sd = ctx.bns
        B, Cin, H, W = ctx.shape
        dev = xr.device
        g = rows_view(nhwc_bf16(gout))
        M1, M2 = y1.shape[0], y3.shape[0]

        def wgrad(conv, dy, x, geom):
            if wants(conv.weight):
                conv_wgrad(dy, x, geom, grad_buffer(conv.weight))
                grads_done(conv.weight)

        dy3 = torch.empty_like(y3)
        dres = torch.empty_like(y3)
        s3.backward(g, y3, out, 3, dy3, dres)
        dyd = None
        if yd is not None:
            dyd = torch.empty_like(yd)
            sd.backward(dres, yd, None, False, dyd, None)
            wgrad(mm.get("downsample")[0], dyd, xr, gd)
        da2 = torch.empty_like(a2)
        conv_dgrad(dy3, g3, w3, da2, w_t=conv1x1_weight_T(mm["conv3"], g3))
        if ctx.probes is not None:
            _fire_grad_hooks(ctx.probes[1], from_rows(da2, B, g2.p, g2.q, g2.k))
        wgrad(mm["conv3"], dy3, a2, g3)
        dy2 = torch.empty_like(y2)
        m1, m2 = ctx.masks if ctx.masks is not None else (None, None)
        s2.backward(da2, y2, m2, 3 if ctx.x3 else 2, dy2, None)
        da1 = torch.empty_like(a1)
        conv_dgrad(dy2, g2, w2, da1, w_flip=None if g2.stride != 1 else
                   conv_weight_flipped(mm["conv2"].weight))
        if ctx.probes is not None:
            _fire_grad_hooks(ctx.probes[0], from_rows(da1, B, g1.p, g1.q, g1.k))
        wgrad(mm["conv2"], dy2, a1, g2)
        dy1 = torch.empty_like(y1)
        s1.backward(da1, y1, m1, 3 if ctx.x3 else 2, dy1, None)
        dx = None
        if ctx.x_requires_grad:
            dxr = _empty((M1, Cin), BF16, dev)
            w1t = conv1x1_weight_T(mm["conv1"], g1)
            if dyd is None:
                conv_dgrad(dy1, g1, w1, dxr, add=dres, w_t=w1t)
            else:
                conv_dgrad(dy1, g1, w1, dxr, w_t=w1t)
                conv_dgrad(dyd, gd, wd, dxr, add=dxr,
                           w_t=conv1x1_weight_T(mm.get("downsample")[0], gd))
            dx = from_rows(dxr, B, H, W, Cin)
        wgrad(mm["conv1"], dy1, xr, g1)
        n_params = len(ctx.needs_input_grad) - 2
        return (dx,) + (None,) * n_params + (None,)


class AvgPoolFn(torch.autograd.Function):
    @staticmethod
    def forward(ctx, x):
        x3 = _take_x3(x) if _x3() and (not _per_stage() or hasattr(x, "_dfu_lo")) else None
        x = nhwc_bf16(x.detach())
        B, C, H, W = x.shape
        ctx.shape = (B, C, H, W)
        if x3 is not None:
            y = ops.avgpool_fwd_x3(x3[0], x3[1], B, H * W, C)
        else:
            y = ops.avgpool_fwd(rows_view(x), B, H * W, C)
        return y.view(B, C, 1, 1)

    @staticmethod
    def backward(ctx, g):
        if g.is_cuda:
            arm_backward_join()
        B, C, H, W = ctx.shape
        g = g.reshape(B, C)
        if g.dtype != F32:
            g = g.float()
        dx = ops.avgpool_bwd(g.contiguous(), B, H * W, C)
        return from_rows(dx.view(B * H * W, C), B, H, W, C)


class PatchEmbedFn(torch.autograd.Function):

    @staticmethod
    def forward(ctx, x, w, b, cls, pos, ps):
        B, C, H, W = x.shape
        D = w.shape[0]
        xf = x.detach().float() if x.dtype != F32 else x.detach()
        T = (H // ps) * (W // ps)
        wb = weight_bf16_rows(w)
        K = wb.shape[1]
        X = _empty((B, T + 1, D), F32, x.device)
        if _x3():
            patches = ops.patchify_f32_x3(xf, ps)
            A, Bop, Kg = patches, weight_x3_rows(w), 3 * K
        else:
            patches = ops.patchify_f32(xf, ps)
            A, Bop, Kg = patches, wb, K
        ops.gemm(B * T, D, Kg, A, Kg, Bop, Kg, X, D, epilogue=L.EPI_PATCH,
                 bias=b.detach() if b is not None else None, aux=pos.detach().reshape(T + 1, D),
                 ldaux=D, ep_tokens=T, x3=Kg != K)
        ops.vit_cls_rows(cls.detach().reshape(D), pos.detach().reshape(T + 1, D), X, B, T + 1, D)
        ctx.params = (w, b, cls, pos)
        ctx.dims = (B, T, D, K, C, H, W, ps)
        ctx.x_requires_grad = ctx.needs_input_grad[0]
        ctx.save_for_backward(patches, wb)
        return X

    @staticmethod
    def backward(ctx, gX):
        patches, wb = ctx.saved_tensors
        w, b, cls, pos = ctx.params
        B, T, D, K, C, H, W, ps = ctx.dims
        gX = gX.contiguous()
        gpatch = ops.vit_embed_bwd(gX, B, T + 1, D,
                                   grad_buffer(cls) if wants(cls) else None,
                                   grad_buffer(pos) if wants(pos) else None,
                                   grad_buffer(b) if wants(b) else None)
        if wants(w):
            dw = grad_buffer(w).view(D, K)
            ops.gemm(D, K, B * T, gpatch, D, patches, patches.stride(0), dw, K,
                     a_mode=L.OPND_MNMAJOR, b_mode=L.OPND_MNMAJOR, epilogue=L.EPI_F32_ACC)
        grads_done(w, b, cls, pos)
        dx = None
        if ctx.x_requires_grad:
            dpatch = _empty((B * T, K), F32, gX.device)
            ops.gemm(B * T, K, D, gpatch, D, wb, K, dpatch, K, b_mode=L.OPND_MNMAJOR,
                     epilogue=L.EPI_F32)
            dx = ops.unpatchify_f32(dpatch, B, C, H, W, ps)
        return dx, None, None, None, None, None


def _linear_wgrad(dy_bf, x_bf, w, rows):
    N, K = w.shape
    ops.gemm(N, K, rows, dy_bf, N, x_bf, x_bf.stride(0), grad_buffer(w), K,
             a_mode=L.OPND_MNMAJOR, b_mode=L.OPND_MNMAJOR, epilogue=L.EPI_F32_ACC)


def _ln_fwd(x2d, norm, rows, D, out_bf):
    mean = _empty((rows,), F32, x2d.device)
    rstd = _empty((rows,), F32, x2d.device)
    ops.layernorm_fwd(x2d, D, rows, D, norm.weight, norm.bias, norm.eps, out_bf, D, True, mean,
                      rstd)
    return mean, rstd


def _ln_bwd(dy_bf, x2d, mean, rstd, norm, rows, D, g, g_bf, gsum=False, batch=None):
    gsp = ops.layernorm_bwd(dy_bf, D, True, x2d, D, mean, rstd, norm.weight, rows, D, g, D, g_bf,
                            grad_buffer(norm.weight) if wants(norm.weight) else None,
                            grad_buffer(norm.bias) if wants(norm.bias) else None, gsum=gsum,
                            batch=batch)
    if batch is None:
        grads_done(norm.weight, norm.bias)
    return gsp


def _colsum_of_grad(g, out, batch=None):
    gsp = getattr(g, "_dfu_colsum", None)
    if gsp is None:
        gsp = ops.colsum_partial(g.reshape(-1, g.shape[-1]))
    if batch is not None:
        batch.add(gsp, out, gsp.shape[1])
    else:
        ops.reduce_partials_add(gsp, out)


def _bf16_of_grad(g):
    gb = getattr(g, "_dfu_bf16", None)
    if gb is not None and gb.shape == g.shape:
        return gb
    return ops.cast_rows_bf16(g.reshape(-1, g.shape[-1])).view(g.shape)


def _linear_dgrad(rows, N, K, g, weight, w_rows, out, epilogue=L.EPI_BF16, **kw):
    wT = weight_bf16_T(weight)
    if wT is not None:
        ops.gemm(rows, N, K, g, K, wT, K, out, N, epilogue=epilogue, **kw)
    else:
        ops.gemm(rows, N, K, g, K, w_rows, N, out, N, b_mode=L.OPND_MNMAJOR, epilogue=epilogue,
                 **kw)


_X3_TILE = int(os.environ.get("DFU_X3_TILE", "8"))
_NO_T192 = os.environ.get("DFU_GEMM_NO_T192", "0") != "0"


def _t768():
    return 9 if _concurrent_encoders[0] == 0 and not _NO_T192 else 0

_DGELU_COLSUM = int(os.environ.get("DFU_DGELU_COLSUM", "2"))


class ViTBlockFn(torch.autograd.Function):

    @staticmethod
    def forward(ctx, x, *params_and_mod):
        blk = params_and_mod[-1]
        bm = blk._modules
        attn, mlp = bm["attn"], bm["mlp"]
        B, T, D = x.shape
        rows = B * T
        H = attn.num_heads
        dh = D // H
        dev = x.device
        x = x.detach().contiguous()
        x2 = x.view(rows, D)
        wqkv = weight_bf16_rows(params_and_mod[2])
        wproj = weight_bf16_rows(params_and_mod[4])
        wfc1 = weight_bf16_rows(params_and_mod[8])
        wfc2 = weight_bf16_rows(params_and_mod[10])
        Dh = wfc1.shape[0]
        bias = lambda lin: lin.bias.detach() if lin.bias is not None else None
        mode = stage_mode(blk)
        if mode == "bf16x3":
            return ViTBlockFn._forward_x3(ctx, blk, x2, B, T, D, H, dh, rows, wqkv, wproj, wfc1,
                                          wfc2, bias)
        if mode == "fp16":
            return ViTBlockFn._forward_h16(ctx, blk, x2, B, T, D, H, dh, rows, wqkv, wproj, wfc1,
                                           wfc2, bias)
        xn1 = _empty((rows, D), BF16, dev)
        m1, r1 = _ln_fwd(x2, blk.norm1, rows, D, xn1)
        qkv = _empty((rows, 3 * D), BF16, dev)
        ops.gemm(rows, 3 * D, D, xn1, D, wqkv, D, qkv, 3 * D, epilogue=L.EPI_BF16,
                 bias=bias(attn.qkv))
        o, lse = ops.attention_fwd(qkv, B, T, H, dh, attn.scale)
        xm = _empty((rows, D), F32, dev)
        t768 = _t768()
        ops.gemm(rows, D, D, o, D, wproj, D, xm, D, epilogue=L.EPI_F32_RESID, bias=bias(attn.proj),
                 aux=x2, ldaux=D, tile=t768)
        xn2 = _empty((rows, D), BF16, dev)
        m2, r2 = _ln_fwd(xm, blk.norm2, rows, D, xn2)
        dgl = _empty((rows, Dh), BF16, dev)
        h = _empty((rows, Dh), BF16, dev)
        ops.gemm(rows, Dh, D, xn2, D, wfc1, D, h, Dh, epilogue=L.EPI_BF16_GELU, bias=bias(mlp.fc1),
                 aux_out=dgl, ldaux_out=Dh)
        xo = _empty((B, T, D), F32, dev)
        ops.gemm(rows, D, Dh, h, Dh, wfc2, Dh, xo.view(rows, D), D, epilogue=L.EPI_F32_RESID,
                 bias=bias(mlp.fc2), aux=xm, ldaux=D, tile=t768)
        ctx.t768 = t768
        ctx.blk = blk
        ctx.dims = (B, T, D, H, dh, Dh)
        ctx.out_ref = weakref.ref(xo)
        ctx.beside = _VIT_WGRAD_STREAM and _concurrent_encoders[0] == 0
        ctx.save_for_backward(x2, xn1, m1, r1, qkv, o, lse, xm, xn2, m2, r2, dgl, h, wqkv,
                              wproj, wfc1, wfc2)
        return xo

    @staticmethod
    def _forward_x3(ctx, blk, x2, B, T, D, H, dh, rows, wqkv, wproj, wfc1, wfc2, bias):
        attn, mlp = blk.attn, blk.mlp
        dev = x2.device
        Dh = wfc1.shape[0]

        def ln_x3(xsrc, norm):
            t3 = _empty((rows, 3 * D), BF16, dev)
            tb = _empty((rows, D), BF16, dev)
            mean = _empty((rows,), F32, dev)
            rstd = _empty((rows,), F32, dev)
            ops.layernorm_fwd_x3(xsrc, D, rows, D, norm.weight, norm.bias, norm.eps, t3, tb, mean,
                                 rstd)
            return t3, tb, mean, rstd

        tl = _X3_TILE
        tl_d = (_t768() or tl) if tl == 8 else tl
        ctx.t768 = _t768()
        xn1_3, xn1, m1, r1 = ln_x3(x2, blk.norm1)
        qkvf = _empty((rows, 3 * D), F32, dev)
        ops.gemm(rows, 3 * D, 3 * D, xn1_3, 3 * D, weight_x3_rows(attn.qkv.weight), 3 * D, qkvf,
                 3 * D, epilogue=L.EPI_F32, bias=bias(attn.qkv), tile=tl, x3=True)
        del xn1_3
        qkv = _empty((rows, 3 * D), BF16, dev)
        o3, o, lse = ops.attention_fwd_f32(qkvf, B, T, H, dh, attn.scale, qkv_bf16=qkv)
        del qkvf
        xm = _empty((rows, D), F32, dev)
        ops.gemm(rows, D, 3 * D, o3, 3 * D, weight_x3_rows(attn.proj.weight), 3 * D, xm, D,
                 epilogue=L.EPI_F32_RESID, bias=bias(attn.proj), aux=x2, ldaux=D, tile=tl_d,
                 x3=True)
        del o3
        xn2_3, xn2, m2, r2 = ln_x3(xm, blk.norm2)
        dgl = _empty((rows, Dh), BF16, dev)
        if tl == 8:
            h3 = _empty((rows, 3 * Dh), BF16, dev)
            ops.gemm(rows, Dh, 3 * D, xn2_3, 3 * D, weight_x3_rows(mlp.fc1.weight), 3 * D, h3,
                     3 * Dh, epilogue=L.EPI_X3_GELU, bias=bias(mlp.fc1), aux_out=dgl,
                     ldaux_out=Dh, tile=tl, x3=True)
            h = h3[:, :Dh]
        else:
            hf = _empty((rows, Dh), F32, dev)
            ops.gemm(rows, Dh, 3 * D, xn2_3, 3 * D, weight_x3_rows(mlp.fc1.weight), 3 * D, hf,
                     Dh, epilogue=L.EPI_F32, bias=bias(mlp.fc1), tile=tl, x3=True)
            h3, h, dgl = ops.gelu_x3(hf)
            del hf
        del xn2_3
        xo = _empty((B, T, D), F32, dev)
        ops.gemm(rows, D, 3 * Dh, h3, 3 * Dh, weight_x3_rows(mlp.fc2.weight), 3 * Dh,
                 xo.view(rows, D), D, epilogue=L.EPI_F32_RESID, bias=bias(mlp.fc2), aux=xm,
                 ldaux=D, tile=tl_d, x3=True)
        ctx.blk = blk
        ctx.dims = (B, T, D, H, dh, Dh)
        ctx.out_ref = weakref.ref(xo)
        ctx.beside = _VIT_WGRAD_STREAM and _concurrent_encoders[0] == 0
        ctx.save_for_backward(x2, xn1, m1, r1, qkv, o, lse, xm, xn2, m2, r2, dgl, h, wqkv,
                              wproj, wfc1, wfc2)
        return xo

    @staticmethod
    def _forward_h16(ctx, blk, x2, B, T, D, H, dh, rows, wqkv, wproj, wfc1, wfc2, bias):
        bm = blk._modules
        attn, mlp = bm["attn"], bm["mlp"]
        am, mm = attn._modules, mlp._modules
        dev = x2.device
        Dh = wfc1.shape[0]
        F16 = torch.float16

        def ln(xsrc, norm):
            t16 = _empty((rows, D), F16, dev)
            tb = _empty((rows, D), BF16, dev)
            mean = _empty((rows,), F32, dev)
            rstd = _empty((rows,), F32, dev)
            ops.layernorm_fwd_h16(xsrc, D, rows, D, norm.weight, norm.bias, norm.eps, t16, tb,
                                  mean, rstd)
            return t16, tb, mean, rstd

        h16 = L.OPERAND_F16
        ctx.t768 = _t768()
        tl_d = ctx.t768 or 8
        xn1_16, xn1, m1, r1 = ln(x2, bm["norm1"])
        qkv = _empty((rows, 3 * D), F16, dev)
        ops.gemm(rows, 3 * D, D, xn1_16, D, weight_f16_rows(am["qkv"].weight), D, qkv, 3 * D,
                 epilogue=L.EPI_F16_DUAL, bias=bias(am["qkv"]), tile=8, operand_type=h16)
        del xn1_16
        o16, o, lse = ops.attention_fwd_f16(qkv, B, T, H, dh, attn.scale)
        xm = _empty((rows, D), F32, dev)
        ops.gemm(rows, D, D, o16, D, weight_f16_rows(am["proj"].weight), D, xm, D,
                 epilogue=L.EPI_F32_RESID, bias=bias(am["proj"]), aux=x2, ldaux=D, tile=tl_d,
                 operand_type=h16)
        del o16
        xn2_16, xn2, m2, r2 = ln(xm, bm["norm2"])
        h2 = _empty((rows, 2 * Dh), BF16, dev)
        dgl = _empty((rows, Dh), BF16, dev)
        ops.gemm(rows, Dh, D, xn2_16, D, weight_f16_rows(mm["fc1"].weight), D, h2, 2 * Dh,
                 epilogue=L.EPI_F16_GELU, bias=bias(mm["fc1"]), aux_out=dgl, ldaux_out=Dh, tile=8,
                 operand_type=h16)
        del xn2_16
        h = h2[:, Dh:]
        xo = _empty((B, T, D), F32, dev)
        ops.gemm(rows, D, Dh, h2, 2 * Dh, weight_f16_rows(mm["fc2"].weight), Dh, xo.view(rows, D),
                 D, epilogue=L.EPI_F32_RESID, bias=bias(mm["fc2"]), aux=xm, ldaux=D, tile=tl_d,
                 operand_type=h16)
        ctx.blk = blk
        ctx.dims = (B, T, D, H, dh, Dh)
        ctx.out_ref = weakref.ref(xo)
        ctx.beside = _VIT_WGRAD_STREAM and _concurrent_encoders[0] == 0
        ctx.save_for_backward(x2, xn1, m1, r1, qkv, o, lse, xm, xn2, m2, r2, dgl, h, wqkv,
                              wproj, wfc1, wfc2)
# ... 268 lines not shown
```

### dfu-multimodal_amd/dfu_hip/ops.py

```python
import ctypes

import torch

from . import _lib as L
from ._lib import check
from .streams import (TILE_COUNTERS, current_stream, on_stream, refuse_in_capture,
                      stream_ptr, stream_wait, tile_counters)

BF16 = torch.bfloat16
F32 = torch.float32
F16 = torch.float16


def lib():
    return L.load()


def ptr(t):
    return None if t is None else t.data_ptr()


def _req(t, dtype, name):
    if t.dtype != dtype:
        raise TypeError(f"{name}: expected {dtype}, got {t.dtype}")
    if not t.is_cuda:
        raise ValueError(f"{name}: tensor must be on the GPU")


class ConvGeom:

    __slots__ = ("n", "h", "w", "c", "k", "r", "s", "stride", "pad", "p", "q")

    def __init__(self, n, h, w, c, k, r, s, stride, pad):
        self.n, self.h, self.w, self.c, self.k = n, h, w, c, k
        self.r, self.s, self.stride, self.pad = r, s, stride, pad
        self.p = (h + 2 * pad - r) // stride + 1
        self.q = (w + 2 * pad - s) // stride + 1


TILES = {"auto": 0, "128x128": 1, "256x128": 2, "128x256": 3, "256x256": 4, "128x128o2": 5,
         "128x128w4": 6, "256x256p8": 7, "256x256ps": 8, "192x256ps": 9, "256x64": 10,
         "128x64o2": 11}

gemm_record = None


def _algorithmic_bytes(d, conv):
    M, N, K = d.M, d.N, d.K
    act_in = 2 * conv.n * conv.h * conv.w * conv.c if conv is not None else 0
    a = {L.OPND_CONV_FWD: act_in,
         L.OPND_CONV_DGRAD: 2 * conv.n * conv.p * conv.q * conv.k if conv is not None else 0
         }.get(d.a_mode, 2 * M * K)
    if d.a_seg and not d.x3_pairs:
        a = a * 2 // 3
    b = act_in if d.b_mode == L.OPND_CONV_WGRAD_X else 2 * N * K
    e = d.epilogue
    c = {L.EPI_F32: 4, L.EPI_F32_RESID: 8, L.EPI_F32_ACC: 8, L.EPI_PATCH: 4, L.EPI_F32_STATS: 4,
         L.EPI_BF16_GELU: 4, L.EPI_BF16_DGELU: 4, L.EPI_BF16_ADD: 4,
         L.EPI_X3_GELU: 8, L.EPI_F16_GELU: 6,
         L.EPI_F16_DUAL: 4 if d.aux_out else 2}.get(e, 2) * M * N
    return a + b + c


def gemm_replay(records, stream=None):
    s = stream_ptr() if stream is None else stream
    fn = lib().dfu_gemm
    for r in records:
        check(fn(ctypes.byref(r[0]), s), "dfu_gemm replay")


def gemm(M, N, K, A, lda, B, ldb, C, ldc, a_mode=L.OPND_KMAJOR, b_mode=L.OPND_KMAJOR,
         epilogue=L.EPI_BF16, alpha=1.0, bias=None, aux=None, ldaux=0, aux_out=None,
         ldaux_out=0, stats=None, split_k=0, ep_tokens=0, conv=None, tile=0, workspace=None,
         operand_type=0, x3=False, a_lo=None, x3_pairs=False):
    for t, name in ((A, "A"), (B, "B"), (C, "C")):
        if not t.is_cuda:
            raise ValueError(f"gemm: operand {name} must be on the GPU (there is no host path)")
    d = L.GemmDesc()
    d.M, d.N, d.K = int(M), int(N), int(K)
    d.a_mode, d.b_mode = int(a_mode), int(b_mode)
    d.A, d.lda = A.data_ptr(), int(lda)
    d.B, d.ldb = B.data_ptr(), int(ldb)
    d.C, d.ldc = C.data_ptr(), int(ldc)
    d.epilogue, d.alpha = int(epilogue), float(alpha)
    d.bias = bias.data_ptr() if bias is not None else None
    d.aux = aux.data_ptr() if aux is not None else None
    d.ldaux = int(ldaux)
    d.aux_out = aux_out.data_ptr() if aux_out is not None else None
    d.ldaux_out = int(ldaux_out)
    d.stats = stats.data_ptr() if stats is not None else None
    d.operand_type = int(operand_type)
    if a_lo is not None:
        nseg = 2 if x3_pairs else 3
        d.a_seg = int(conv.c // nseg if a_mode == L.OPND_CONV_FWD else K // nseg)
        d.a_lo = a_lo.data_ptr()
        d.x3_pairs = int(bool(x3_pairs))
    d.split_k = int(split_k)
    d.ep_tokens = int(ep_tokens)
    d.tile = int(tile)
    if conv is not None:
        d.conv_n, d.conv_h, d.conv_w, d.conv_c = conv.n, conv.h, conv.w, conv.c
        d.conv_k, d.conv_r, d.conv_s = conv.k, conv.r, conv.s
        d.conv_stride, d.conv_pad, d.conv_p, d.conv_q = conv.stride, conv.pad, conv.p, conv.q
    lb = lib()
    ref = ctypes.byref(d)
    need = lb.dfu_gemm_workspace_bytes(ref)
    if need > 0:
        if workspace is None or workspace.numel() * workspace.element_size() < need:
            workspace = torch.empty(need, dtype=torch.uint8, device=C.device)
        d.workspace = workspace.data_ptr()
        d.workspace_bytes = int(need)
        cnt = tile_counters(C.device)
        d.tile_counters, d.tile_counters_len = cnt.data_ptr(), cnt.numel()
    rc = lb.dfu_gemm(ref, stream_ptr())
    if rc:
        check(rc, "dfu_gemm")
    if gemm_record is not None:
        flops = 2.0 * M * N * (K // (2 if x3_pairs else 3) if x3 else K)
        if a_mode == L.OPND_CONV_DGRAD and conv is not None:
            flops /= conv.stride * conv.stride
        executed = 3.0 * flops if x3 else 2.0 * M * N * K
        gemm_record.append((d, flops, _algorithmic_bytes(d, conv),
                            (A, B, C, bias, aux, aux_out, stats, workspace, a_lo), executed))


def gemm_set_tail_split(enable):
    return int(lib().dfu_gemm_set_tail_split(int(bool(enable))))


def gemm_set_inkernel_reduce(enable):
    return int(lib().dfu_gemm_set_inkernel_reduce(int(bool(enable))))


def _plan_desc(M, N, K, a_mode, b_mode, epilogue, split_k, tile):
    d = L.GemmDesc()
    d.M, d.N, d.K = int(M), int(N), int(K)
    d.a_mode, d.b_mode, d.epilogue = int(a_mode), int(b_mode), int(epilogue)
    d.split_k, d.tile = int(split_k), int(tile)
    return d


def gemm_workspace_bytes(M, N, K, a_mode, b_mode, epilogue=L.EPI_F32_ACC, split_k=0, tile=0):
    d = _plan_desc(M, N, K, a_mode, b_mode, epilogue, split_k, tile)
    return int(lib().dfu_gemm_workspace_bytes(ctypes.byref(d)))


def gemm_plan(M, N, K, a_mode, b_mode, epilogue, split_k=0, tile=0):
    d = _plan_desc(M, N, K, a_mode, b_mode, epilogue, split_k, tile)
    t, sk = ctypes.c_int32(), ctypes.c_int32()
    check(lib().dfu_gemm_plan(ctypes.byref(d), ctypes.byref(t), ctypes.byref(sk)), "dfu_gemm_plan")
    return t.value, sk.value


PERSISTENT_ALL = 3


def gemm_set_persistent(mode):
    return int(lib().dfu_gemm_set_persistent(int(mode)))


def gemm_f32(M, N, K, A, sam, sak, B, sbn, sbk, C, ldc, bias=None, relu=False, accumulate=False):
    need = lib().dfu_gemm_f32_workspace_bytes(int(M), int(N), int(K))
    ws = torch.empty(need, dtype=torch.uint8, device=C.device) if need > 0 else None
    check(lib().dfu_gemm_f32(int(M), int(N), int(K), ptr(A), int(sam), int(sak), ptr(B), int(sbn),
                             int(sbk), ptr(C), int(ldc), ptr(bias), int(relu), int(accumulate),
                             ptr(ws), int(need), stream_ptr()), "dfu_gemm_f32")


def stats_tiles(M):
    return lib().dfu_gemm_stats_tiles(int(M))


def pack_conv_weight(w, out=None):
    _req(w, F32, "pack_conv_weight")
    K, C, R, S = w.shape
    if out is None:
        out = torch.empty((K, R, S, C), dtype=BF16, device=w.device)
    check(lib().dfu_pack_conv_weight(ptr(w.contiguous()), ptr(out), K, C, R, S, stream_ptr()),
          "dfu_pack_conv_weight")
    return out


def conv_grad_krsc_to_oihw(krsc, oihw):
    K, C, R, S = oihw.shape
    check(lib().dfu_conv_grad_krsc_to_oihw(ptr(krsc), ptr(oihw), K, C, R, S, stream_ptr()),
          "dfu_conv_grad_krsc_to_oihw")


def cast_rows_bf16(x, ld_out=None, out=None):
    _req(x, F32, "cast_rows_bf16")
    x2 = x.reshape(-1, x.shape[-1])
    if x2.stride(1) != 1:
        x2 = x2.contiguous()
    rows, cols = x2.shape
    ld_out = cols if ld_out is None else ld_out
    if out is None:
        out = torch.empty((rows, ld_out), dtype=BF16, device=x.device)
    check(lib().dfu_cast_rows_bf16(ptr(x2), x2.stride(0), ptr(out), ld_out, rows, cols,
                                   stream_ptr()), "dfu_cast_rows_bf16")
    return out


def cast_rows_f16(x, ld_out=None, out=None):
    _req(x, F32, "cast_rows_f16")
    x2 = x.reshape(-1, x.shape[-1])
    if x2.stride(1) != 1:
        x2 = x2.contiguous()
    rows, cols = x2.shape
    ld_out = cols if ld_out is None else ld_out
    if out is None:
        out = torch.empty((rows, ld_out), dtype=F16, device=x.device)
    check(lib().dfu_cast_rows_f16(ptr(x2), x2.stride(0), ptr(out), ld_out, rows, cols,
                                  stream_ptr()), "dfu_cast_rows_f16")
    return out


class TransposeJobs:

    def __init__(self, pairs):
        import struct
        raw, tile0 = bytearray(), 0
        for src, dst in pairs:
            _req(src, BF16, "transpose_bf16")
            _req(dst, BF16, "transpose_bf16")
            r, c = src.shape
            ok = (dst.shape == (c, r) and r % 8 == 0 and c % 8 == 0 and src.stride(1) == 1 and
                  dst.stride(1) == 1 and src.stride(0) % 8 == 0 and dst.stride(0) % 8 == 0 and
                  src.data_ptr() % 16 == 0 and dst.data_ptr() % 16 == 0)
            if not ok:
                raise ValueError(f"transpose_bf16: [{r}, {c}] stride {src.stride()} -> "
                                 f"{tuple(dst.shape)} stride {dst.stride()} unsupported")
            raw += struct.pack("<QQiiiiii", src.data_ptr(), dst.data_ptr(), r, c, tile0,
                               src.stride(0), dst.stride(0), 0)
            tile0 += ((r + 63) // 64) * ((c + 63) // 64)
        self.pairs = list(pairs)
        self.njobs, self.ntiles = len(self.pairs), tile0
        dev = self.pairs[0][0].device
        self.table = torch.frombuffer(bytearray(raw), dtype=torch.uint8).to(dev)

    def launch(self):
        check(lib().dfu_transpose_bf16(ptr(self.table), self.njobs, self.ntiles, stream_ptr()),
              "dfu_transpose_bf16")


def transpose_bf16(src, out=None):
    if out is None:
        out = torch.empty((src.shape[1], src.shape[0]), dtype=BF16, device=src.device)
    TransposeJobs([(src, out)]).launch()
    return out


def cast_rows_f32(x, out=None):
    _req(x, BF16, "cast_rows_f32")
    x2 = x.reshape(-1, x.shape[-1])
    rows, cols = x2.shape
    if out is None:
        out = torch.empty((rows, cols), dtype=F32, device=x.device)
    check(lib().dfu_cast_rows_f32(ptr(x2), x2.stride(0), ptr(out), out.stride(0), rows, cols,
                                  stream_ptr()), "dfu_cast_rows_f32")
    return out


def im2col_f32(x, R, S, stride, pad, Kp):
    _req(x, F32, "im2col_f32")
    B, C, H, W = x.shape
    P = (H + 2 * pad - R) // stride + 1
    Q = (W + 2 * pad - S) // stride + 1
    out = torch.empty((B * P * Q, Kp), dtype=BF16, device=x.device)
    sn, sc, sh, sw = x.stride()
    check(lib().dfu_im2col_f32(ptr(x), sn, sc, sh, sw, B, C, H, W, R, S, stride, pad, P, Q,
                               ptr(out), Kp, stream_ptr()), "dfu_im2col_f32")
    return out, P, Q


def patchify_f32(x, ps):
    _req(x, F32, "patchify_f32")
    B, C, H, W = x.shape
    out = torch.empty((B * (H // ps) * (W // ps), C * ps * ps), dtype=BF16, device=x.device)
    sn, sc, sh, sw = x.stride()
    check(lib().dfu_patchify_f32(ptr(x), sn, sc, sh, sw, B, C, H, W, ps, ptr(out),
                                 stream_ptr()), "dfu_patchify_f32")
    return out


def col2im_f32(dcol, B, C, H, W, R, S, stride, pad, P, Q, Kp):
    _req(dcol, F32, "col2im_f32")
    dx = torch.empty((B, C, H, W), dtype=F32, device=dcol.device)
    check(lib().dfu_col2im_f32(ptr(dcol), B, C, H, W, R, S, stride, pad, P, Q, Kp, ptr(dx),
                               stream_ptr()), "dfu_col2im_f32")
    return dx


def unpatchify_f32(dpatch, B, C, H, W, ps):
    _req(dpatch, F32, "unpatchify_f32")
    dx = torch.empty((B, C, H, W), dtype=F32, device=dpatch.device)
    check(lib().dfu_unpatchify_f32(ptr(dpatch), B, C, H, W, ps, ptr(dx), stream_ptr()),
          "dfu_unpatchify_f32")
    return dx


def gradcam(act, grad):
    if act.dtype not in (BF16, F32) or not act.is_cuda or not grad.is_cuda:
        raise TypeError("gradcam: bf16/fp32 CUDA tensors expected")
    grad = grad.to(act.dtype)
    B, Ca, h, w = act.shape
    Bg, Cg, hg, wg = grad.shape
    if (B, h, w) != (Bg, hg, wg):
        raise ValueError(f"gradcam: activation {tuple(act.shape)} vs gradient {tuple(grad.shape)}")
    views = []
    for t in (act, grad):
        if t.stride(2) != w * t.stride(3):
            t = t.contiguous(memory_format=torch.channels_last)
        views.append((t, t.stride(0), t.stride(3), t.stride(1)))
    (a, sab, sap, sac), (g, sgb, sgp, sgc) = views
    cam = torch.empty((B, h, w), dtype=F32, device=act.device)
    check(lib().dfu_gradcam(ptr(a), Ca, sab, sap, sac, ptr(g), Cg, sgb, sgp, sgc,
                            int(a.dtype == BF16), B, h * w, ptr(cam), stream_ptr()), "dfu_gradcam")
    return cam


def saliency(dx):
    _req(dx, F32, "saliency")
    dx = dx.contiguous()
    B, C, H, W = dx.shape
    out = torch.empty((B, H, W), dtype=F32, device=dx.device)
    check(lib().dfu_saliency(ptr(dx), B, C, H * W, ptr(out), stream_ptr()), "dfu_saliency")
    return out


def _slice_ws(nbytes, device):
    if nbytes <= 0:
        return None, None
    return torch.empty(nbytes // 8, dtype=torch.float64, device=device), tile_counters(device)


def bn_finalize(stats, M, C, gamma, beta, eps, momentum, running_mean, running_var, nbt,
                mean_out, invstd_out, scale_out, shift_out):
    tiles = stats_tiles(M)
    ws, cnt = _slice_ws(lib().dfu_bn_finalize_ws_bytes(tiles, C), stats.device)
    check(lib().dfu_bn_finalize(ptr(stats), tiles, M, C, ptr(gamma), ptr(beta), eps, momentum,
                                ptr(running_mean), ptr(running_var), ptr(nbt), ptr(mean_out),
                                ptr(invstd_out), ptr(scale_out), ptr(shift_out), ptr(ws), ptr(cnt),
                                0 if cnt is None else cnt.numel(), stream_ptr()),
          "dfu_bn_finalize")


def bn_eval_coeffs(gamma, beta, rm, rv, eps, scale_out, shift_out):
    check(lib().dfu_bn_eval_coeffs(ptr(gamma), ptr(beta), ptr(rm), ptr(rv), eps, rm.numel(),
                                   ptr(scale_out), ptr(shift_out), stream_ptr()),
          "dfu_bn_eval_coeffs")


def bn_tile_stats(x, M, C):
    _req(x, BF16, "bn_tile_stats")
    stats = torch.empty((stats_tiles(M), 2, C), dtype=F32, device=x.device)
    check(lib().dfu_bn_tile_stats(ptr(x), int(M), int(C), ptr(stats), stream_ptr()),
          "dfu_bn_tile_stats")
    return stats


def bn_apply(y, scale, shift, residual, relu, out, M, C, mask=None):
    if mask is None:
        check(lib().dfu_bn_apply(ptr(y), ptr(scale), ptr(shift), ptr(residual), int(relu),
                                 ptr(out), M, C, stream_ptr()), "dfu_bn_apply")
    else:
        check(lib().dfu_bn_apply_mask(ptr(y), ptr(scale), ptr(shift), ptr(residual), int(relu),
                                      ptr(out), ptr(mask), M, C, stream_ptr()),
              "dfu_bn_apply_mask")


_BN_BWD_WS = {}


def bn_bwd(dout, y, out, relu, mean, invstd, gamma, M, C, dy, dres, dgamma, dbeta,
           batch_stats=True, scale=None, shift=None):
    relu = int(relu)
    if relu == 2 and (scale is None or shift is None):
        raise ValueError("bn_bwd: relu=2 needs the forward scale/shift")
    lb = lib()
    nb = _BN_BWD_WS.get((M, C))
    if nb is None:
        nb = _BN_BWD_WS[(M, C)] = int(lb.dfu_bn_bwd_ws_bytes(M, C))
    dev = y.device
    ws = torch.empty((nb + 7) // 8, dtype=torch.float64, device=dev)
    cnt = tile_counters(dev)
    rc = lb.dfu_bn_bwd(ptr(dout), y.data_ptr(), ptr(out), relu, ptr(scale), ptr(shift),
                       mean.data_ptr(), invstd.data_ptr(), ptr(gamma), M, C, int(batch_stats),
                       ptr(dgamma), ptr(dbeta), dy.data_ptr(), ptr(dres), ws.data_ptr(), nb,
                       cnt.data_ptr(), cnt.numel(), stream_ptr())
    if rc:
        check(rc, "dfu_bn_bwd")


def maxpool_fwd(x, B, H, W, C, scale=None, shift=None):
    P = (H - 1) // 2 + 1
    Q = (W - 1) // 2 + 1
    y = torch.empty((B, P, Q, C), dtype=BF16, device=x.device)
    am = torch.empty((B, P, Q, C), dtype=torch.uint8, device=x.device)
    if scale is None:
        check(lib().dfu_maxpool_fwd(ptr(x), B, H, W, C, ptr(y), ptr(am), P, Q, stream_ptr()),
              "dfu_maxpool_fwd")
    else:
        check(lib().dfu_maxpool_bn_fwd(ptr(x), ptr(scale), ptr(shift), B, H, W, C, ptr(y),
                                       ptr(am), P, Q, stream_ptr()), "dfu_maxpool_bn_fwd")
    return y, am, P, Q


def maxpool_bwd(dy, am, B, H, W, C, P, Q):
    dx = torch.empty((B, H, W, C), dtype=BF16, device=dy.device)
    check(lib().dfu_maxpool_bwd(ptr(dy), ptr(am), B, H, W, C, P, Q, ptr(dx), stream_ptr()),
          "dfu_maxpool_bwd")
    return dx


def avgpool_fwd(x, B, HW, C):
    y = torch.empty((B, C), dtype=F32, device=x.device)
    check(lib().dfu_avgpool_fwd(ptr(x), B, HW, C, ptr(y), stream_ptr()), "dfu_avgpool_fwd")
    return y


def avgpool_bwd(dy, B, HW, C):
    dx = torch.empty((B, HW, C), dtype=BF16, device=dy.device)
    check(lib().dfu_avgpool_bwd(ptr(dy), B, HW, C, ptr(dx), stream_ptr()), "dfu_avgpool_bwd")
    return dx


def layernorm_fwd(x, ldx, rows, D, gamma, beta, eps, out, ldo, out_bf16, mean, rstd):
    check(lib().dfu_layernorm_fwd(ptr(x), ldx, rows, D, ptr(gamma), ptr(beta), eps, ptr(out),
# ... 466 lines not shown
```

### include/dfu_hip.h

```cpp
#ifndef DFU_HIP_H
#define DFU_HIP_H
#include <stdint.h>

#ifdef __cplusplus
extern "C" {
#endif

#define DFU_OK 0
#define DFU_E_INVALID 1001
#define DFU_E_UNSUPPORTED 1002

const char* dfu_last_error_string(void);
int dfu_version(void);
int dfu_zero(void* ptr, int64_t bytes, void* stream);

int dfu_stream_create(int32_t priority, void** stream);
int dfu_stream_destroy(void* stream);
int dfu_stream_wait(void* waiter, void* producer);
int dfu_stream_capture_status(void* stream, int32_t* status);
int dfu_streams_abort_capture(void* const* streams, int32_t n, int32_t* still_capturing);

enum dfu_operand_mode {
  DFU_OPND_KMAJOR = 0,
  DFU_OPND_MNMAJOR = 1,
  DFU_OPND_CONV_FWD = 2,
  DFU_OPND_CONV_DGRAD = 3,
  DFU_OPND_CONV_DGRAD_W = 4,
  DFU_OPND_CONV_WGRAD_X = 5
};
enum dfu_epilogue {
  DFU_EPI_BF16 = 0,
  DFU_EPI_BF16_RELU = 1,
  DFU_EPI_BF16_GELU = 2,
  DFU_EPI_F32 = 3,
  DFU_EPI_F32_RESID = 4,
  DFU_EPI_BF16_DGELU = 5,
  DFU_EPI_BF16_ADD = 6,
  DFU_EPI_F32_ACC = 7,
  DFU_EPI_F32_ACC_CONVW = 8,
  DFU_EPI_BF16_STATS = 9,
  DFU_EPI_PATCH = 10,
  DFU_EPI_F32_STATS = 11,
  DFU_EPI_BF16_DSTATS = 12,
  DFU_EPI_X3_GELU = 13,
  DFU_EPI_F16_DUAL = 14,
  DFU_EPI_F16_GELU = 15
};

typedef struct dfu_gemm_desc {
  int32_t M, N, K;
  int32_t a_mode, b_mode;
  const void* A;
  int64_t lda;
  const void* B;
  int64_t ldb;
  void* C;
  int64_t ldc;
  int32_t epilogue;
  float alpha;
  const float* bias;
  const void* aux;
  int64_t ldaux;
  void* aux_out;
  int64_t ldaux_out;
  float* stats;
  int32_t split_k;
  int32_t ep_tokens;
  int32_t conv_n, conv_h, conv_w, conv_c;
  int32_t conv_k, conv_r, conv_s;
  int32_t conv_stride, conv_pad;
  int32_t conv_p, conv_q;
  int32_t tile;
  void* workspace;
  int64_t workspace_bytes;
  int32_t* tile_counters;
  int32_t tile_counters_len;
  int32_t operand_type;
  int32_t a_seg;
  const void* a_lo;
  int32_t x3_pairs;
} dfu_gemm_desc;

int dfu_gemm(const dfu_gemm_desc* desc, void* stream);
int dfu_gemm_stats_tiles(int32_t M);
int64_t dfu_gemm_workspace_bytes(const dfu_gemm_desc* desc);
int dfu_gemm_plan(const dfu_gemm_desc* desc, int32_t* tile, int32_t* split_k);
int dfu_gemm_set_persistent(int32_t mode);
int dfu_gemm_set_inkernel_reduce(int32_t enable);
int dfu_gemm_set_tail_split(int32_t enable);
int dfu_gemm_f32(int32_t M, int32_t N, int32_t K, const float* A, int64_t sam, int64_t sak,
                 const float* B, int64_t sbn, int64_t sbk, float* C, int64_t ldc,
                 const float* bias, int32_t relu, int32_t accumulate, void* workspace,
                 int64_t workspace_bytes, void* stream);
int64_t dfu_gemm_f32_workspace_bytes(int32_t M, int32_t N, int32_t K);

int dfu_pack_conv_weight(const float* w, void* out_bf16, int32_t K, int32_t C, int32_t R,
                         int32_t S, void* stream);
int dfu_conv_grad_krsc_to_oihw(const float* krsc, float* oihw, int32_t K, int32_t C, int32_t R,
                               int32_t S, void* stream);
int dfu_cast_rows_bf16(const float* in, int64_t ld_in, void* out, int64_t ld_out, int32_t rows,
                       int32_t cols, void* stream);
typedef struct dfu_transpose_job {
  const void* src;
  void* dst;
  int32_t rows, cols;
  int32_t tile0;
  int32_t ld_src, ld_dst;
  int32_t pad_;
} dfu_transpose_job;
int dfu_transpose_bf16(const dfu_transpose_job* jobs, int32_t njobs, int32_t ntiles,
                       void* stream);
int dfu_cast_rows_f16(const float* in, int64_t ld_in, void* out, int64_t ld_out, int32_t rows,
                      int32_t cols, void* stream);
int dfu_cast_rows_f32(const void* in, int64_t ld_in, float* out, int64_t ld_out, int32_t rows,
                      int32_t cols, void* stream);
int dfu_im2col_f32(const float* x, int64_t sn, int64_t sc, int64_t sh, int64_t sw, int32_t B,
                   int32_t C, int32_t H, int32_t W, int32_t R, int32_t S, int32_t stride,
                   int32_t pad, int32_t P, int32_t Q, void* out, int32_t Kp, void* stream);
int dfu_patchify_f32(const float* x, int64_t sn, int64_t sc, int64_t sh, int64_t sw, int32_t B,
                     int32_t C, int32_t H, int32_t W, int32_t ps, void* out, void* stream);

int dfu_col2im_f32(const float* dcol, int32_t B, int32_t C, int32_t H, int32_t W, int32_t R,
                   int32_t S, int32_t stride, int32_t pad, int32_t P, int32_t Q, int32_t Kp,
                   float* dx, void* stream);
int dfu_unpatchify_f32(const float* dpatch, int32_t B, int32_t C, int32_t H, int32_t W,
                       int32_t ps, float* dx, void* stream);
int dfu_gradcam(const void* act, int32_t Ca, int64_t sab, int64_t sap, int64_t sac,
                const void* grad, int32_t Cg, int64_t sgb, int64_t sgp, int64_t sgc,
                int32_t is_bf16, int32_t B, int32_t HW, float* cam, void* stream);
int dfu_saliency(const float* dx, int32_t B, int32_t C, int32_t HW, float* out, void* stream);

int dfu_bn_finalize(const float* stats, int32_t tiles, int32_t M, int32_t C, const float* gamma,
                    const float* beta, float eps, float momentum, float* running_mean,
                    float* running_var, int64_t* num_batches, float* mean_out,
                    float* invstd_out, float* scale_out, float* shift_out, double* ws,
                    int32_t* counters, int32_t ncounters, void* stream);
int64_t dfu_bn_finalize_ws_bytes(int32_t tiles, int32_t C);
int dfu_bn_tile_stats(const void* x, int64_t M, int32_t C, float* stats, void* stream);
int dfu_bn_eval_coeffs(const float* gamma, const float* beta, const float* running_mean,
                       const float* running_var, float eps, int32_t C, float* scale_out,
                       float* shift_out, void* stream);
int dfu_bn_apply(const void* y, const float* scale, const float* shift, const void* residual,
                 int32_t relu, void* out, int64_t M, int32_t C, void* stream);
int dfu_bn_apply_mask(const void* y, const float* scale, const float* shift,
                      const void* residual, int32_t relu, void* out, uint8_t* mask, int64_t M,
                      int32_t C, void* stream);
int dfu_bn_bwd_blocks(int64_t M, int32_t C);
int dfu_bn_bwd_reduce(const void* dout, const void* y, const void* out, int32_t relu,
                      const float* scale, const float* shift, const float* mean,
                      const float* invstd, int64_t M, int32_t C, float* partial, void* stream);
int dfu_bn_bwd_finalize(const float* partial, int32_t blocks, int64_t M, int32_t C,
                        const float* gamma, const float* invstd, int32_t batch_stats,
                        float* dgamma, float* dbeta, float* coef, double* ws, int32_t* counters,
                        int32_t ncounters, void* stream);
int64_t dfu_bn_bwd_finalize_ws_bytes(int32_t blocks, int32_t C);
int dfu_bn_bwd_apply(const void* dout, const void* y, const void* out, int32_t relu,
                     const float* scale, const float* shift, const float* mean,
                     const float* invstd, const float* coef, int64_t M, int32_t C, void* dy,
                     void* dres, void* stream);
int64_t dfu_bn_bwd_ws_bytes(int64_t M, int32_t C);
int dfu_bn_bwd(const void* dout, const void* y, const void* out, int32_t relu, const float* scale,
               const float* shift, const float* mean, const float* invstd, const float* gamma,
               int64_t M, int32_t C, int32_t batch_stats, float* dgamma, float* dbeta, void* dy,
               void* dres, void* ws, int64_t ws_bytes, int32_t* counters, int32_t ncounters,
               void* stream);

int dfu_maxpool_fwd(const void* x, int32_t B, int32_t H, int32_t W, int32_t C, void* y,
                    uint8_t* argmax, int32_t P, int32_t Q, void* stream);
int dfu_maxpool_bn_fwd(const void* x, const float* scale, const float* shift, int32_t B,
                       int32_t H, int32_t W, int32_t C, void* y, uint8_t* argmax, int32_t P,
                       int32_t Q, void* stream);
int dfu_maxpool_bwd(const void* dy, const uint8_t* argmax, int32_t B, int32_t H, int32_t W,
                    int32_t C, int32_t P, int32_t Q, void* dx, void* stream);
int dfu_avgpool_fwd(const void* x, int32_t B, int32_t HW, int32_t C, float* y, void* stream);
int dfu_avgpool_bwd(const float* dy, int32_t B, int32_t HW, int32_t C, void* dx, void* stream);

int dfu_layernorm_fwd(const float* x, int64_t ldx, int32_t rows, int32_t D, const float* gamma,
                      const float* beta, float eps, void* out, int64_t ldo, int32_t out_bf16,
                      float* mean, float* rstd, void* stream);
int dfu_ln_bwd_blocks(int32_t rows);
int dfu_layernorm_bwd(const void* dy, int64_t lddy, int32_t dy_bf16, const float* x,
                      int64_t ldx, const float* mean, const float* rstd, const float* gamma,
                      int32_t rows, int32_t D, float* gx, int64_t ldg, void* gx_bf16,
                      float* partial, float* gsum_partial, void* stream);
int dfu_reduce_partials(const float* partial, int32_t blocks, int32_t nvec, int32_t D,
                        float* out0, float* out1, void* stream);
#define DFU_REDUCE_BATCH 8
typedef struct dfu_reduce_entry {
  const float* partial;
  int64_t stride;
  float* out;
  int32_t blocks;
  int32_t D;
} dfu_reduce_entry;
int dfu_reduce_partials_batch(const dfu_reduce_entry* entries, int32_t n, void* stream);

int dfu_attention_fwd(const void* qkv, int32_t B, int32_t N, int32_t H, int32_t dh, float scale,
                      void* o, float* lse, void* stream);
int dfu_attention_fwd_f16(const void* qkv, int32_t B, int32_t N, int32_t H, int32_t dh,
                          float scale, void* o, void* o_bf16, float* lse, void* stream);
int dfu_attention_bwd(const void* qkv, const void* o, const void* dout, const float* lse,
                      int32_t B, int32_t N, int32_t H, int32_t dh, float scale, float* delta,
                      void* dqkv, void* stream);
int dfu_attention_bwd_qkv16(const void* qkv16, const void* o, const void* dout, const float* lse,
                            int32_t B, int32_t N, int32_t H, int32_t dh, float scale,
                            float* delta, void* dqkv, void* stream);
int dfu_attention_npad(int32_t N);

int dfu_vit_cls_rows(const float* cls, const float* pos, float* x, int32_t B, int32_t T,
                     int32_t D, void* stream);
int dfu_vit_embed_bwd(const float* gx, int32_t B, int32_t T, int32_t D, float* dcls,
                      float* dpos, float* dbias, void* gpatch, float* partial, void* stream);

int dfu_colsum(const void* x, int32_t is_bf16, int64_t ld, int32_t rows, int32_t N, float* out,
               float* partial, void* stream);
int dfu_colsum_blocks(int32_t rows);
int dfu_gather_rows_f32(const float* in, int64_t ld_in, int32_t stride, int32_t offset,
                        int32_t rows, int32_t D, float* out, int64_t ld_out, void* stream);
int dfu_scatter_rows_f32(const float* in, int64_t ld_in, int32_t stride, int32_t offset,
                         int32_t rows, int32_t D, float* out, int64_t ld_out, void* stream);
int dfu_relu_fwd(const void* x, void* y, int64_t n, int32_t is_bf16, void* stream);
int dfu_relu_bwd(const void* dy, const void* y, void* dx, int64_t n, int32_t is_bf16,
                 void* stream);
int dfu_dropout_fwd(const void* x, void* y, uint8_t* mask, int64_t n, float p, uint64_t seed,
                    int64_t* offset_dev, int32_t is_bf16, void* stream);
int dfu_dropout_bwd(const void* dy, const uint8_t* mask, void* dx, int64_t n, float p,
                    int32_t is_bf16, void* stream);
int dfu_concat2_bf16(const void* a, int32_t a_bf16, int32_t Na, const void* b, int32_t b_bf16,
                     int32_t Nb, int32_t rows, void* out, void* stream);
int dfu_split2_f32(const void* g, int32_t g_bf16, int32_t rows, int32_t Na, int32_t Nb,
                   float* ga, float* gb, void* stream);

int dfu_ce_weighted_fwd(const float* logits, const int64_t* labels, const float* weight,
                        int32_t B, int32_t C, float* loss, float* dlogits, void* stream);
int dfu_ce_weighted_bwd(const float* dlogits_saved, const float* grad_loss, int32_t B,
                        int32_t C, float* dlogits, void* stream);
int dfu_adamw(float* const* params, float* const* grads, float* const* exp_avg,
              float* const* exp_avg_sq, const int64_t* numels, int32_t ntensors,
              const int64_t* chunk_offsets, int32_t nchunks, float lr, float beta1,
              float beta2, float eps, float weight_decay, int64_t* step_dev, void* stream);
int dfu_adamw_flat(float* param, const float* grad, float* exp_avg, float* exp_avg_sq, int64_t n,
                   float lr, float beta1, float beta2, float eps, float weight_decay,
                   const int64_t* step_dev, void* shadow_bf16, void* shadow_f16, void* shadow_x3,
                   int64_t x3_begin, int64_t x3_end, void* stream);
int dfu_step_increment(int64_t* step_dev, void* stream);
int dfu_argmax_rows(const float* x, int32_t rows, int32_t C, int64_t* out, void* stream);
int dfu_softmax_rows(const float* x, int32_t rows, int32_t C, float* out, void* stream);
int dfu_metrics_accumulate(const float* logits, const int64_t* labels, int32_t rows, int32_t C,
                           const float* loss, int64_t* confusion, double* loss_sum,
                           int64_t* batches, void* stream);

int dfu_split_x3(const float* in, int64_t ld_in, int32_t rows, int32_t cols, int32_t seg,
                 void* out, int32_t pattern, void* hi_out, int64_t ld_hi, void* stream);
int dfu_pack_conv_weight_x3(const float* w, void* out, int32_t K, int32_t C, int32_t R, int32_t S,
                            int32_t pattern, void* stream);
int dfu_im2col_f32_x3(const float* x, int64_t sn, int64_t sc, int64_t sh, int64_t sw, int32_t B,
                      int32_t C, int32_t H, int32_t W, int32_t R, int32_t S, int32_t stride,
                      int32_t pad, int32_t P, int32_t Q, void* out, void* out_lo, int32_t Kp,
                      void* stream);
int dfu_patchify_f32_x3(const float* x, int64_t sn, int64_t sc, int64_t sh, int64_t sw, int32_t B,
                        int32_t C, int32_t H, int32_t W, int32_t ps, void* out, void* stream);
int dfu_bn_apply_x3(const void* y, const void* y_lo, const float* scale, const float* shift,
                    const void* residual, const void* residual_lo, int32_t res_mode, int32_t relu,
                    void* out_lo, void* out_bf16, float* out_f32, void* y_bf16,
                    uint8_t* relu_mask, int64_t M, int32_t C, void* stream);
int dfu_maxpool_fwd_x3(const float* x, int32_t B, int32_t H, int32_t W, int32_t C, void* y_lo,
                       void* y_bf16, uint8_t* argmax, int32_t P, int32_t Q, void* stream);
int dfu_stem_conv_x3(const float* x, int64_t sn, int64_t sc, int64_t sh, int64_t sw, int32_t B,
                     int32_t C, int32_t H, int32_t W, const float* w, int32_t K, int32_t R,
                     int32_t S, int32_t stride, int32_t pad, void* y, void* y_lo, float* stats,
                     void* col, void* stream);
int64_t dfu_stem_wgrad_ws_bytes(int32_t B, int32_t H, int32_t W);
int dfu_stem_wgrad_x3(const float* x, int64_t sn, int64_t sc, int64_t sh, int64_t sw, int32_t B,
                      int32_t C, int32_t H, int32_t W, const void* dy, int32_t K, int32_t R,
                      int32_t S, int32_t stride, int32_t pad, float* dw, float* slab,
                      int64_t slab_bytes, void* stream);
int dfu_maxpool_bn_fwd_x3(const void* y, const void* y_lo, const float* scale, const float* shift,
                          int32_t B, int32_t H, int32_t W, int32_t C, void* out_lo,
                          void* out_bf16, uint8_t* argmax, uint8_t* relu_mask, int32_t P,
                          int32_t Q, void* stream);
int dfu_avgpool_fwd_x3(const void* hi, const void* lo, int32_t B, int32_t HW, int32_t C, float* y,
                       void* stream);
int dfu_layernorm_fwd_x3(const float* x, int64_t ldx, int32_t rows, int32_t D,
                         const float* gamma, const float* beta, float eps, void* out3,
                         void* out_bf16, float* mean, float* rstd, void* stream);
int dfu_layernorm_fwd_h16(const float* x, int64_t ldx, int32_t rows, int32_t D,
                          const float* gamma, const float* beta, float eps, void* out_f16,
                          void* out_bf16, float* mean, float* rstd, void* stream);
int dfu_gelu_x3(const float* hpre, int64_t rows, int32_t N, void* h3, void* h_bf16,
                void* dgelu_bf16, void* stream);
int dfu_attention_fwd_f32(const float* qkv, int32_t B, int32_t N, int32_t H, int32_t dh,
                          float scale, int32_t npad, void* qkv_bf16, void* o3, void* o_bf16,
                          float* lse, void* stream);

typedef struct dfu_resize_desc {
  int64_t src_off;
  int64_t tmp_off;
  int64_t coef_off;
  int32_t w, h;
  int32_t ksh, ksv;
} dfu_resize_desc;

enum dfu_aug_op { DFU_AUG_BRIGHTNESS = 0, DFU_AUG_CONTRAST = 1, DFU_AUG_SATURATION = 2 };

typedef struct dfu_aug_params {
  int32_t hflip, vflip;
  int32_t rotate;
  int32_t rot[6];
  int32_t affine;
  int32_t aff[6];
  int32_t n_ops;
  int32_t op[3];
  float factor[3];
} dfu_aug_params;

int dfu_resize_ksize(int32_t in_size, int32_t out_size);
int dfu_resize_coeffs(int32_t in_size, int32_t out_size, int32_t* bounds, int32_t* kk);
int dfu_resize_batch(const uint8_t* src, const dfu_resize_desc* descs, const int32_t* coefs,
                     int32_t n, int32_t out_w, int32_t out_h, uint8_t* tmp, uint8_t* dst,
                     void* stream);
int dfu_augment_normalize(const uint8_t* img, const dfu_aug_params* params, int32_t n,
                          int32_t H, int32_t W, const float* mean3, const float* std3,
                          int32_t* contrast_means, float* out, void* stream);

enum dfu_aug_order { DFU_AUG_ORDER_FLIP_ROTATE = 0, DFU_AUG_ORDER_ROTATE_FLIP = 1 };
int dfu_augment_views(const uint8_t* img, int32_t n_images, const dfu_aug_params* params,
                      const int32_t* view_src, int32_t n_views, int32_t order, int32_t H,
                      int32_t W, const float* mean3, const float* std3, int32_t* contrast_means,
                      float* out, void* stream);
int dfu_tta_reduce(const float* logits, int32_t samples, int32_t views, int32_t C,
                   float* prob_out, int64_t* pred_out, void* stream);
int dfu_binary_eval_counts(const float* prob, const int64_t* pred, const int64_t* labels,
                           int32_t n, int64_t* counts, void* stream);

#ifdef __cplusplus
}
#endif
#endif
```

Measured before the change: 3154.

## Batch ResNet bottleneck weight-gradient GEMMs into one grouped split-K launch

Adds a grouped GEMM kernel that runs up to four weight-gradient GEMMs of a bottleneck block in a single launch, with a shared split-K plan and one fused slab-reduction kernel. The GEMM kernel body is factored out so the group kernel can dispatch per member on the 128x128 occupancy-2 tile. The ResNet bottleneck backward now collects its conv wgrads and issues them together, enabled by default. This targets launch overhead and poor CU fill on small wgrad GEMMs. In exchange it fixes the tile choice, allocates a workspace on every call, and delays when the gradients become ready for overlap.

```diff
diff --git a/dfu-multimodal_amd/csrc/gemm.hip b/dfu-multimodal_amd/csrc/gemm.hip
--- a/dfu-multimodal_amd/csrc/gemm.hip
+++ b/dfu-multimodal_amd/csrc/gemm.hip
@@ -623,3 +623,22 @@
 }
 
 }
+
+int dfu::gemm_group_member_args(const dfu_gemm_desc* d, int split, float* slab, GemmArgs* a) {
+  dfu_gemm_desc m = *d;
+  m.tile = T128x128o2 + 1;
+  m.split_k = split;
+  m.tile_counters = nullptr;
+  m.tile_counters_len = 0;
+  m.workspace = slab;
+  m.workspace_bytes = slab ? (int64_t)split * d->M * d->N * 4 : 0;
+  Plan pl;
+  int rc = check_desc(&m, true, &pl);
+  if (rc != DFU_OK) return rc;
+  fill_args(&m, pl, nullptr, *a);
+  rc = check_ranges(&m, pl, nullptr, *a);
+  if (rc != DFU_OK) return rc;
+  a->tail_full = a->tail_r = a->tail_s = a->tail_kps = 0;
+  a->tslab = nullptr;
+  return DFU_OK;
+}
diff --git a/dfu-multimodal_amd/csrc/gemm_group.hip b/dfu-multimodal_amd/csrc/gemm_group.hip
--- /dev/null
+++ b/dfu-multimodal_amd/csrc/gemm_group.hip
@@ -0,0 +1,222 @@
+#include <limits.h>
+#include <stdlib.h>
+
+#include "gemm_table.h"
+
+using namespace dfu;
+
+namespace {
+
+constexpr int kMaxMembers = 4;
+constexpr int kCUs = 256;
+using GT = Tile<128, 128, 2>;
+
+inline int cdiv(int a, int b) { return (a + b - 1) / b; }
+inline int64_t align256(int64_t x) { return (x + 255) & ~(int64_t)255; }
+
+struct GroupArgs {
+  GemmArgs m[kMaxMembers];
+  int first[kMaxMembers + 1];
+  int conv_b[kMaxMembers];
+};
+
+__global__ __launch_bounds__(GT::NT, GT::OCC) void k_gemm_group(const GroupArgs g) {
+  __shared__ __attribute__((aligned(16))) char smem[GT::LDS_BYTES + 16];
+  const int u = blockIdx.x;
+  int mi = 0;
+#pragma unroll
+  for (int i = 1; i < kMaxMembers; ++i) mi += u >= g.first[i] ? 1 : 0;
+  const GemmArgs& p = g.m[mi];
+  const int bid = u - g.first[mi], nwg = g.first[mi + 1] - g.first[mi];
+  if (g.conv_b[mi])
+    gemm_body<DFU_OPND_MNMAJOR, DFU_OPND_CONV_WGRAD_X, DFU_EPI_F32_ACC, GT::TM, GT::TN, GT::OCC>(
+        p, smem, bid, nwg);
+  else
+    gemm_body<DFU_OPND_MNMAJOR, DFU_OPND_MNMAJOR, DFU_EPI_F32_ACC, GT::TM, GT::TN, GT::OCC>(
+        p, smem, bid, nwg);
+}
+
+struct ReduceMember {
+  const float* slab;
+  float* C;
+  int64_t ldc;
+  int M, N, split;
+  int first;
+};
+struct ReduceArgs {
+  ReduceMember m[kMaxMembers];
+  int first_end[kMaxMembers];
+};
+
+__global__ __launch_bounds__(1024) void k_group_reduce(const ReduceArgs g) {
+  __shared__ f32x4 red[16][64];
+  const int lane = threadIdx.x & 63, w = threadIdx.x >> 6, nw = blockDim.x >> 6;
+  const int b = blockIdx.x;
+  int mi = 0;
+#pragma unroll
+  for (int i = 0; i < kMaxMembers - 1; ++i) mi += b >= g.first_end[i] ? 1 : 0;
+  const ReduceMember& r = g.m[mi];
+  const int64_t units = (int64_t)r.M * r.N / 4;
+  const int64_t e = (int64_t)(b - r.first) * 64 + lane;
+  f32x4 s = {0.f, 0.f, 0.f, 0.f};
+  if (e < units) {
+    const f32x4* p = (const f32x4*)r.slab + e;
+#pragma unroll 4
+    for (int k = w; k < r.split; k += nw) s += p[k * units];
+  }
+  red[w][lane] = s;
+  __syncthreads();
+  if (w != 0 || e >= units) return;
+  for (int j = 1; j < nw; ++j) s += red[j][lane];
+  const int64_t m = 4 * e / r.N;
+  const int n = (int)(4 * e - m * r.N);
+  f32x4* c = (f32x4*)(r.C + m * r.ldc + n);
+  *c += s;
+}
+
+struct TileRow {
+  int occ;
+  double step_us, round_us;
+};
+#define X(name, tm, tn, occ, phased, tail_ok, step_us, round_us) {occ, step_us, round_us},
+const TileRow kRows[NTILES] = {DFU_TILES(X)};
+#undef X
+const TileRow& kRow = kRows[T128x128o2];
+constexpr double kSlabGBs = 5000.0, kReduceLaunchUs = 2.0;
+constexpr int kMinSteps = 24;
+
+struct MemberPlan {
+  int tiles, ktiles, split;
+  int64_t slab_off;
+};
+struct GroupPlan {
+  MemberPlan m[kMaxMembers];
+  int units = 0;
+  int max_split = 1;
+  int64_t ws_bytes = 0;
+};
+
+inline int eff_split(int ktiles, int s) { return cdiv(ktiles, cdiv(ktiles, s < 1 ? 1 : s)); }
+
+int check_members(const dfu_gemm_desc* d, int n, const char* who) {
+  DFU_CHECK_ARG(d != nullptr && n >= 1 && n <= kMaxMembers, "%s: 1..%d members (got %d)", who,
+                kMaxMembers, n);
+  for (int i = 0; i < n; ++i) {
+    const dfu_gemm_desc& m = d[i];
+    DFU_CHECK_ARG(m.M > 0 && m.N > 0 && m.K > 0, "%s: member %d: bad shape", who, i);
+    DFU_CHECK_ARG(m.a_mode == DFU_OPND_MNMAJOR &&
+                      (m.b_mode == DFU_OPND_MNMAJOR || m.b_mode == DFU_OPND_CONV_WGRAD_X) &&
+                      m.epilogue == DFU_EPI_F32_ACC && m.operand_type == 0 && m.a_seg == 0,
+                  "%s: member %d: weight-gradient form only (MN-major A, MN-major or "
+                  "CONV_WGRAD_X B, F32_ACC, bf16)", who, i);
+    DFU_CHECK_ARG(m.N % 4 == 0 && m.ldc % 4 == 0, "%s: member %d: N and ldc %% 4", who, i);
+  }
+  return DFU_OK;
+}
+
+GroupPlan plan_group(const dfu_gemm_desc* d, int n, int force_split) {
+  GroupPlan g;
+  int kmax = 1;
+  for (int i = 0; i < n; ++i) {
+    g.m[i].tiles = cdiv(d[i].M, GT::TM) * cdiv(d[i].N, GT::TN);
+    g.m[i].ktiles = cdiv(d[i].K, BK);
+    if (g.m[i].ktiles > kmax) kmax = g.m[i].ktiles;
+  }
+  int best_kps = kmax;
+  const char* fixed = getenv("DFU_GEMM_GROUP_KPS");
+  if (force_split <= 0 && fixed != nullptr && atoi(fixed) > 0) {
+    best_kps = atoi(fixed);
+  } else if (force_split <= 0) {
+    double best = 1e30;
+    const int smax = kmax < 256 ? kmax : 256;
+    const int slots = kCUs * kRow.occ;
+    bool filled = false;
+    for (int s = 1; s <= smax; ++s) {
+      const int kps = cdiv(kmax, s);
+      if (kps < kMinSteps && filled) break;
+      int64_t units = 0;
+      double slab_us = 0.0;
+      for (int i = 0; i < n; ++i) {
+        const int se = eff_split(g.m[i].ktiles, cdiv(g.m[i].ktiles, kps));
+        units += (int64_t)g.m[i].tiles * se;
+        if (se > 1) slab_us += 4.0 * (se + 2) * (double)d[i].M * d[i].N / (kSlabGBs * 1e3);
+      }
+      const double rounds = (double)((units + slots - 1) / slots);
+      const double cost = rounds * (kRow.round_us + kps * kRow.step_us) + slab_us +
+                          (slab_us > 0.0 ? kReduceLaunchUs : 0.0);
+      if (cost < best) {
+        best = cost;
+        best_kps = kps;
+      }
+      filled = filled || units >= slots;
+    }
+  }
+  for (int i = 0; i < n; ++i) {
+    MemberPlan& m = g.m[i];
+    m.split = eff_split(m.ktiles, force_split > 0 ? force_split : cdiv(m.ktiles, best_kps));
+    m.slab_off = g.ws_bytes;
+    if (m.split > 1) g.ws_bytes += align256((int64_t)m.split * d[i].M * d[i].N * 4);
+    if (m.split > g.max_split) g.max_split = m.split;
+    g.units += m.tiles * m.split;
+  }
+  return g;
+}
+
+}
+
+extern "C" int64_t dfu_gemm_group_ws_bytes(const dfu_gemm_desc* members, int32_t n,
+                                           int32_t force_split) {
+  if (check_members(members, n, "dfu_gemm_group_ws_bytes") != DFU_OK) return -1;
+  return plan_group(members, n, force_split).ws_bytes;
+}
+
+extern "C" int dfu_gemm_group(const dfu_gemm_desc* members, int32_t n, void* workspace,
+                              int64_t workspace_bytes, int32_t force_split, void* stream) {
+  int rc = check_members(members, n, "dfu_gemm_group");
+  if (rc != DFU_OK) return rc;
+  DFU_CHECK_ARG(force_split >= 0, "dfu_gemm_group: force_split must be >= 0 (0 = plan)");
+  const GroupPlan gp = plan_group(members, n, force_split);
+  DFU_CHECK_ARG(gp.ws_bytes == 0 || (workspace != nullptr && workspace_bytes >= gp.ws_bytes &&
+                                     ((uintptr_t)workspace & 15) == 0),
+                "dfu_gemm_group: workspace of %lld bytes, need %lld (dfu_gemm_group_ws_bytes), "
+                "16-byte aligned", (long long)workspace_bytes, (long long)gp.ws_bytes);
+  GroupArgs ga;
+  ReduceArgs ra;
+  int first = 0, rfirst = 0;
+  for (int i = 0; i < kMaxMembers; ++i) {
+    ga.first[i] = ga.first[i + 1] = INT_MAX;
+    ga.conv_b[i] = 0;
+    ra.first_end[i] = INT_MAX;
+    ra.m[i] = ReduceMember{nullptr, nullptr, 0, 0, 4, 1, 0};
+    if (i >= n) ga.m[i] = ga.m[0];
+    if (i >= n) continue;
+    const dfu_gemm_desc& d = members[i];
+    const MemberPlan& mp = gp.m[i];
+    DFU_CHECK_ARG(((uintptr_t)d.C & 15) == 0, "dfu_gemm_group: member %d: C 16-byte aligned", i);
+    float* slab = mp.split > 1 ? (float*)((char*)workspace + mp.slab_off) : nullptr;
+    rc = gemm_group_member_args(&d, mp.split, slab, &ga.m[i]);
+    if (rc != DFU_OK) return rc;
+    DFU_CHECK_ARG(ga.m[i].split == mp.split && (mp.split == 1) == (ga.m[i].slab == nullptr),
+                  "dfu_gemm_group: member %d: plan mismatch", i);
+    ga.conv_b[i] = d.b_mode == DFU_OPND_CONV_WGRAD_X;
+    ga.first[i] = first;
+    first += mp.tiles * mp.split;
+    ra.m[i] = ReduceMember{slab, (float*)d.C, d.ldc, d.M, d.N, mp.split, rfirst};
+    if (mp.split > 1) rfirst += (int)(((int64_t)d.M * d.N / 4 + 63) / 64);
+  }
+  for (int i = 0; i < n; ++i) {
+    ga.first[i + 1] = i + 1 < n ? ga.first[i + 1] : first;
+    ra.first_end[i] = i + 1 < n ? ra.m[i + 1].first : rfirst;
+  }
+  for (int i = n + 1; i <= kMaxMembers; ++i) ga.first[i] = INT_MAX;
+  for (int i = n; i < kMaxMembers; ++i) ra.first_end[i] = INT_MAX;
+  hipStream_t s = (hipStream_t)stream;
+  hipLaunchKernelGGL(k_gemm_group, dim3(first), dim3(GT::NT), 0, s, ga);
+  DFU_LAUNCH_CHECK();
+  if (rfirst > 0) {
+    const int nw = gp.max_split < 16 ? gp.max_split : 16;
+    hipLaunchKernelGGL(k_group_reduce, dim3(rfirst), dim3(64 * nw), 0, s, ra);
+    DFU_LAUNCH_CHECK();
+  }
+  return DFU_OK;
+}
diff --git a/dfu-multimodal_amd/csrc/gemm_kernel.h b/dfu-multimodal_amd/csrc/gemm_kernel.h
--- a/dfu-multimodal_amd/csrc/gemm_kernel.h
+++ b/dfu-multimodal_amd/csrc/gemm_kernel.h
@@ -859,205 +859,25 @@
 template <int AMODE, int BMODE, int EPI, int TM, int TN, int OCC = 1, int NST = 0, int NW = 8,
           bool X3 = false>
 __global__ __launch_bounds__(64 * NW, OCC) void gemm_kernel(const GemmArgs p) {
-  using T = Tile<TM, TN, OCC, NST, NW>;
-  constexpr int WGN = T::WGN, WTM = T::WTM, WTN = T::WTN;
-  constexpr int FM = T::FM, FN = T::FN, NSTAGE = T::NSTAGE;
-  constexpr int SCRATCH = (EPI == DFU_EPI_BF16_STATS || EPI == DFU_EPI_F32_STATS)
-                              ? T::STATS_BYTES
-                              : 16;
-  __shared__ __attribute__((aligned(16))) char smem[T::LDS_BYTES + SCRATCH];
-  const int tid = threadIdx.x;
-  const int lane = tid & 63;
-  const int wave = tid >> 6;
-  const int wr = wave / WGN, wc = wave % WGN;
-
-  constexpr bool kTail = NW == 8 && FM * FN <= 8 && EPI != DFU_EPI_F32_ACC;
-  const int tiles = p.tiles_m * p.tiles_n;
-  const int units = kTail && p.tail_r ? p.tail_full + p.tail_r * p.tail_s : tiles * p.split;
-  const int nwg = gridDim.x;
-  const int bid = blockIdx.x;
-  int wg = bid;
-  if (nwg >= 16) {
-    const int xcd = bid & 7, q = nwg >> 3, r = nwg & 7;
-    wg = (xcd < r ? xcd * (q + 1) : r * (q + 1) + (xcd - r) * q) + (bid >> 3);
-  }
-  const int full = units / nwg;
-  const int rounds = full + (bid < units - full * nwg ? 1 : 0);
-  if (rounds == 0) return;
-  auto unit_at = [&](int i) { return i * nwg + (i < full ? wg : bid); };
-
-  auto unit_geom = [&](int u, int& m0, int& n0, int& kb, int& nk) {
-    constexpr int GROUP_M = 4;
-    int s, t, kps;
-    if (kTail && p.tail_r && u >= p.tail_full) {
-      const int v = u - p.tail_full;
-      s = v / p.tail_r;
-      t = p.tail_full + (v - s * p.tail_r);
-      kps = p.tail_kps;
-    } else {
-      s = u / tiles;
-      t = u - s * tiles;
-      kps = p.kt_per_split;
-    }
-    const int band = GROUP_M * p.tiles_n;
-    const int g0 = (t / band) * GROUP_M;
-    const int gm = min(GROUP_M, p.tiles_m - g0);
-    const int within = t - (t / band) * band;
-    m0 = (g0 + within % gm) * TM;
-    n0 = (within / gm) * TN;
-    kb = s * kps;
-    nk = min(p.ktiles, kb + kps) - kb;
-  };
-  int total = 0;
-  for (int i = 0; i < rounds; ++i) {
-    int m0_, n0_, kb_, nk_;
-    unit_geom(unit_at(i), m0_, n0_, kb_, nk_);
-    total += nk_;
-  }
-
-  LoadState<T::NLDA> sa;
-  LoadState<T::NLDB> sb;
-  int iu = 0, ik = 0, im0, in0, ikb, ink;
-  unit_geom(unit_at(0), im0, in0, ikb, ink);
-  load_init<AMODE, T::NLDA, NW>(p, sa, p.A, p.lda, im0, p.M, tid);
-  load_init<BMODE, T::NLDB, NW>(p, sb, p.B, p.ldb, in0, p.N, tid);
-  auto issue_next = [&](char* stage) {
-    if (!(p.dbg & 4)) {
-    issue_tile<AMODE, T::NLDA, NW, true, X3>(p, sa, p.A, p.lda, p.m_ld_bound, ikb + ik, p.K, tid,
-                                         stage);
-    issue_tile<BMODE, T::NLDB, NW>(p, sb, p.B, p.ldb, p.n_ld_bound, ikb + ik, p.K, tid,
-                               stage + T::A_BYTES);
-    }
-    if (++ik == ink) {
-      ik = 0;
-      if (++iu < rounds) {
-        unit_geom(unit_at(iu), im0, in0, ikb, ink);
-        load_init<AMODE, T::NLDA, NW>(p, sa, p.A, p.lda, im0, p.M, tid);
-        load_init<BMODE, T::NLDB, NW>(p, sb, p.B, p.ldb, in0, p.N, tid);
-      }
-    }
-  };
-
-  f32x4 acc[FM][FN];
-#pragma unroll
-  for (int i = 0; i < FM; ++i)
-#pragma unroll
-    for (int j = 0; j < FN; ++j) acc[i][j] = (f32x4){0.f, 0.f, 0.f, 0.f};
-
-  constexpr bool AK = kcontig<AMODE>();
-  constexpr bool BKc = kcontig<BMODE>();
-  auto compute = [&](const char* la) {
-    const char* lb = la + T::A_BYTES;
-    static_assert(!X3 || (FM * FN < 32 && AK && BKc),
-                  "interleaved pairs: K-contiguous operands, at most 64x64 per wave");
-    if constexpr (FM * FN >= 32) {
-#pragma unroll
-      for (int ks = 0; ks < 2; ++ks) {
-        bf16x8 fa[FM], fb[FN];
-#pragma unroll
-        for (int i = 0; i < FM; ++i) fa[i] = read_frag<AK>(la, wr * WTM + i * 16, ks, lane);
-#pragma unroll
-        for (int j = 0; j < FN; ++j) fb[j] = read_frag<BKc>(lb, wc * WTN + j * 16, ks, lane);
-        if constexpr (!AK || !BKc) {
-          lds_reads_retired();
-#pragma unroll
-          for (int i = 0; i < FM; ++i) pin(fa[i]);
-#pragma unroll
-          for (int j = 0; j < FN; ++j) pin(fb[j]);
-        }
-#pragma unroll
-        for (int i = 0; i < FM; ++i)
-#pragma unroll
-          for (int j = 0; j < FN; ++j)
-            acc[i][j] = __builtin_amdgcn_mfma_f32_16x16x32_bf16(fb[j], fa[i], acc[i][j], 0, 0, 0);
-      }
-    } else {
-      bf16x8 fa[2][FM], fb[2][FN];
-#pragma unroll
-      for (int ks = 0; ks < 2; ++ks) {
-#pragma unroll
-        for (int i = 0; i < FM; ++i) fa[ks][i] = read_frag<AK>(la, wr * WTM + i * 16, ks, lane);
-#pragma unroll
-        for (int j = 0; j < FN; ++j) fb[ks][j] = read_frag<BKc>(lb, wc * WTN + j * 16, ks, lane);
-      }
-      __builtin_amdgcn_sched_barrier(0);
-      if constexpr (!AK || !BKc) {
-        lds_reads_retired();
-#pragma unroll
-        for (int ks = 0; ks < 2; ++ks) {
-#pragma unroll
-          for (int i = 0; i < FM; ++i) pin(fa[ks][i]);
-#pragma unroll
-          for (int j = 0; j < FN; ++j) pin(fb[ks][j]);
-        }
-      }
-      if constexpr (X3) {
-#pragma unroll
-        for (int t = 0; t < 3; ++t)
-#pragma unroll
-          for (int i = 0; i < FM; ++i)
-#pragma unroll
-            for (int j = 0; j < FN; ++j)
-              acc[i][j] = __builtin_amdgcn_mfma_f32_16x16x32_bf16(fb[t == 2][j], fa[t == 1][i],
-                                                                 acc[i][j], 0, 0, 0);
-      } else {
-#pragma unroll
-        for (int ks = 0; ks < 2; ++ks)
-#pragma unroll
-          for (int i = 0; i < FM; ++i)
-#pragma unroll
-            for (int j = 0; j < FN; ++j)
-              acc[i][j] =
-                  __builtin_amdgcn_mfma_f32_16x16x32_bf16(fb[ks][j], fa[ks][i], acc[i][j], 0, 0, 0);
-      }
-    }
-  };
-
-  const int E = (p.dbg & 1) ? 0 : epi_stores<EPI, T>(p);
-  AuxPre<T> pre;
-  float* red = (float*)(smem + T::LDS_BYTES);
-  unsigned hist = 0;
-  int ci = 0, cu = unit_at(0), ck = 0, cm0, cn0, ckb, cnk;
-  unit_geom(cu, cm0, cn0, ckb, cnk);
-#pragma unroll
-  for (int s = 0; s < NSTAGE - 1; ++s)
-    if (s < total) issue_next(smem + s * T::STAGE_BYTES);
-  int slot = 0;
-  for (int g = 0; g < total; ++g) {
-    const int later = min(NSTAGE - 2, total - 1 - g);
-    const unsigned win = hist & ((1u << (NSTAGE - 1)) - 1u);
-    if (win == 0 && later == NSTAGE - 2)
-      wait_vmcnt<T::DMA_PER_STAGE * (NSTAGE - 2)>();
-    else
-      wait_vm_le<63>(T::DMA_PER_STAGE * later + E * __builtin_popcount(win));
-    __builtin_amdgcn_s_barrier();
-    if (g + NSTAGE - 1 < total) {
-      const int is = slot == 0 ? NSTAGE - 1 : slot - 1;
-      issue_next(smem + is * T::STAGE_BYTES);
-    }
-    if constexpr (aux_prefetch<EPI, T>())
-      if (ck + 1 == cnk) aux_load<AMODE, EPI, T>(p, cm0, cn0, tid, pre);
-    if (!(p.dbg & 2)) compute(smem + slot * T::STAGE_BYTES);
-    slot = slot == NSTAGE - 1 ? 0 : slot + 1;
-    hist <<= 1;
-    if (++ck == cnk) {
-      bool epi = true;
-      if constexpr (kTail)
-        if (p.tail_r && cu >= p.tail_full) epi = tail_reduce<T>(p, acc, cu - p.tail_full, red, tid);
-      if (epi && !(p.dbg & 1))
-        epilogue<AMODE, EPI, T>(p, acc, cm0, cn0, cu / tiles, red, tid, pre);
-#pragma unroll
-      for (int i = 0; i < FM; ++i)
-#pragma unroll
-        for (int j = 0; j < FN; ++j) acc[i][j] = (f32x4){0.f, 0.f, 0.f, 0.f};
-      hist |= 1u;
-      ck = 0;
-      if (++ci < rounds) {
-        cu = unit_at(ci);
-        unit_geom(cu, cm0, cn0, ckb, cnk);
-      }
-    }
-  }
-}
-
-}
+#define DFU_GEMM_BODY_SMEM __shared__ __attribute__((aligned(16))) char smem[T::LDS_BYTES + SCRATCH]
+#define DFU_GEMM_BODY_NWG gridDim.x
+#define DFU_GEMM_BODY_BID blockIdx.x
+#include "gemm_kernel_body.inc"
+#undef DFU_GEMM_BODY_SMEM
+#undef DFU_GEMM_BODY_NWG
+#undef DFU_GEMM_BODY_BID
+}
+
+template <int AMODE, int BMODE, int EPI, int TM, int TN, int OCC = 1, int NST = 0, int NW = 8,
+          bool X3 = false>
+DFU_DEV void gemm_body(const GemmArgs& p, char* smem_, const int bid_, const int nwg_) {
+#define DFU_GEMM_BODY_SMEM char* const smem = smem_
+#define DFU_GEMM_BODY_NWG nwg_
+#define DFU_GEMM_BODY_BID bid_
+#include "gemm_kernel_body.inc"
+#undef DFU_GEMM_BODY_SMEM
+#undef DFU_GEMM_BODY_NWG
+#undef DFU_GEMM_BODY_BID
+}
+
+}
diff --git a/dfu-multimodal_amd/csrc/gemm_kernel_body.inc b/dfu-multimodal_amd/csrc/gemm_kernel_body.inc
--- /dev/null
+++ b/dfu-multimodal_amd/csrc/gemm_kernel_body.inc
@@ -0,0 +1,199 @@
+  using T = Tile<TM, TN, OCC, NST, NW>;
+  constexpr int WGN = T::WGN, WTM = T::WTM, WTN = T::WTN;
+  constexpr int FM = T::FM, FN = T::FN, NSTAGE = T::NSTAGE;
+  constexpr int SCRATCH = (EPI == DFU_EPI_BF16_STATS || EPI == DFU_EPI_F32_STATS)
+                              ? T::STATS_BYTES
+                              : 16;
+  DFU_GEMM_BODY_SMEM;
+  const int tid = threadIdx.x;
+  const int lane = tid & 63;
+  const int wave = tid >> 6;
+  const int wr = wave / WGN, wc = wave % WGN;
+
+  constexpr bool kTail = NW == 8 && FM * FN <= 8 && EPI != DFU_EPI_F32_ACC;
+  const int tiles = p.tiles_m * p.tiles_n;
+  const int units = kTail && p.tail_r ? p.tail_full + p.tail_r * p.tail_s : tiles * p.split;
+  const int nwg = DFU_GEMM_BODY_NWG;
+  const int bid = DFU_GEMM_BODY_BID;
+  int wg = bid;
+  if (nwg >= 16) {
+    const int xcd = bid & 7, q = nwg >> 3, r = nwg & 7;
+    wg = (xcd < r ? xcd * (q + 1) : r * (q + 1) + (xcd - r) * q) + (bid >> 3);
+  }
+  const int full = units / nwg;
+  const int rounds = full + (bid < units - full * nwg ? 1 : 0);
+  if (rounds == 0) return;
+  auto unit_at = [&](int i) { return i * nwg + (i < full ? wg : bid); };
+
+  auto unit_geom = [&](int u, int& m0, int& n0, int& kb, int& nk) {
+    constexpr int GROUP_M = 4;
+    int s, t, kps;
+    if (kTail && p.tail_r && u >= p.tail_full) {
+      const int v = u - p.tail_full;
+      s = v / p.tail_r;
+      t = p.tail_full + (v - s * p.tail_r);
+      kps = p.tail_kps;
+    } else {
+      s = u / tiles;
+      t = u - s * tiles;
+      kps = p.kt_per_split;
+    }
+    const int band = GROUP_M * p.tiles_n;
+    const int g0 = (t / band) * GROUP_M;
+    const int gm = min(GROUP_M, p.tiles_m - g0);
+    const int within = t - (t / band) * band;
+    m0 = (g0 + within % gm) * TM;
+    n0 = (within / gm) * TN;
+    kb = s * kps;
+    nk = min(p.ktiles, kb + kps) - kb;
+  };
+  int total = 0;
+  for (int i = 0; i < rounds; ++i) {
+    int m0_, n0_, kb_, nk_;
+    unit_geom(unit_at(i), m0_, n0_, kb_, nk_);
+    total += nk_;
+  }
+
+  LoadState<T::NLDA> sa;
+  LoadState<T::NLDB> sb;
+  int iu = 0, ik = 0, im0, in0, ikb, ink;
+  unit_geom(unit_at(0), im0, in0, ikb, ink);
+  load_init<AMODE, T::NLDA, NW>(p, sa, p.A, p.lda, im0, p.M, tid);
+  load_init<BMODE, T::NLDB, NW>(p, sb, p.B, p.ldb, in0, p.N, tid);
+  auto issue_next = [&](char* stage) {
+    if (!(p.dbg & 4)) {
+    issue_tile<AMODE, T::NLDA, NW, true, X3>(p, sa, p.A, p.lda, p.m_ld_bound, ikb + ik, p.K, tid,
+                                         stage);
+    issue_tile<BMODE, T::NLDB, NW>(p, sb, p.B, p.ldb, p.n_ld_bound, ikb + ik, p.K, tid,
+                               stage + T::A_BYTES);
+    }
+    if (++ik == ink) {
+      ik = 0;
+      if (++iu < rounds) {
+        unit_geom(unit_at(iu), im0, in0, ikb, ink);
+        load_init<AMODE, T::NLDA, NW>(p, sa, p.A, p.lda, im0, p.M, tid);
+        load_init<BMODE, T::NLDB, NW>(p, sb, p.B, p.ldb, in0, p.N, tid);
+      }
+    }
+  };
+
+  f32x4 acc[FM][FN];
+#pragma unroll
+  for (int i = 0; i < FM; ++i)
+#pragma unroll
+    for (int j = 0; j < FN; ++j) acc[i][j] = (f32x4){0.f, 0.f, 0.f, 0.f};
+
+  constexpr bool AK = kcontig<AMODE>();
+  constexpr bool BKc = kcontig<BMODE>();
+  auto compute = [&](const char* la) {
+    const char* lb = la + T::A_BYTES;
+    static_assert(!X3 || (FM * FN < 32 && AK && BKc),
+                  "interleaved pairs: K-contiguous operands, at most 64x64 per wave");
+    if constexpr (FM * FN >= 32) {
+#pragma unroll
+      for (int ks = 0; ks < 2; ++ks) {
+        bf16x8 fa[FM], fb[FN];
+#pragma unroll
+        for (int i = 0; i < FM; ++i) fa[i] = read_frag<AK>(la, wr * WTM + i * 16, ks, lane);
+#pragma unroll
+        for (int j = 0; j < FN; ++j) fb[j] = read_frag<BKc>(lb, wc * WTN + j * 16, ks, lane);
+        if constexpr (!AK || !BKc) {
+          lds_reads_retired();
+#pragma unroll
+          for (int i = 0; i < FM; ++i) pin(fa[i]);
+#pragma unroll
+          for (int j = 0; j < FN; ++j) pin(fb[j]);
+        }
+#pragma unroll
+        for (int i = 0; i < FM; ++i)
+#pragma unroll
+          for (int j = 0; j < FN; ++j)
+            acc[i][j] = __builtin_amdgcn_mfma_f32_16x16x32_bf16(fb[j], fa[i], acc[i][j], 0, 0, 0);
+      }
+    } else {
+      bf16x8 fa[2][FM], fb[2][FN];
+#pragma unroll
+      for (int ks = 0; ks < 2; ++ks) {
+#pragma unroll
+        for (int i = 0; i < FM; ++i) fa[ks][i] = read_frag<AK>(la, wr * WTM + i * 16, ks, lane);
+#pragma unroll
+        for (int j = 0; j < FN; ++j) fb[ks][j] = read_frag<BKc>(lb, wc * WTN + j * 16, ks, lane);
+      }
+      __builtin_amdgcn_sched_barrier(0);
+      if constexpr (!AK || !BKc) {
+        lds_reads_retired();
+#pragma unroll
+        for (int ks = 0; ks < 2; ++ks) {
+#pragma unroll
+          for (int i = 0; i < FM; ++i) pin(fa[ks][i]);
+#pragma unroll
+          for (int j = 0; j < FN; ++j) pin(fb[ks][j]);
+        }
+      }
+      if constexpr (X3) {
+#pragma unroll
+        for (int t = 0; t < 3; ++t)
+#pragma unroll
+          for (int i = 0; i < FM; ++i)
+#pragma unroll
+            for (int j = 0; j < FN; ++j)
+              acc[i][j] = __builtin_amdgcn_mfma_f32_16x16x32_bf16(fb[t == 2][j], fa[t == 1][i],
+                                                                 acc[i][j], 0, 0, 0);
+      } else {
+#pragma unroll
+        for (int ks = 0; ks < 2; ++ks)
+#pragma unroll
+          for (int i = 0; i < FM; ++i)
+#pragma unroll
+            for (int j = 0; j < FN; ++j)
+              acc[i][j] =
+                  __builtin_amdgcn_mfma_f32_16x16x32_bf16(fb[ks][j], fa[ks][i], acc[i][j], 0, 0, 0);
+      }
+    }
+  };
+
+  const int E = (p.dbg & 1) ? 0 : epi_stores<EPI, T>(p);
+  AuxPre<T> pre;
+  float* red = (float*)(smem + T::LDS_BYTES);
+  unsigned hist = 0;
+  int ci = 0, cu = unit_at(0), ck = 0, cm0, cn0, ckb, cnk;
+  unit_geom(cu, cm0, cn0, ckb, cnk);
+#pragma unroll
+  for (int s = 0; s < NSTAGE - 1; ++s)
+    if (s < total) issue_next(smem + s * T::STAGE_BYTES);
+  int slot = 0;
+  for (int g = 0; g < total; ++g) {
+    const int later = min(NSTAGE - 2, total - 1 - g);
+    const unsigned win = hist & ((1u << (NSTAGE - 1)) - 1u);
+    if (win == 0 && later == NSTAGE - 2)
+      wait_vmcnt<T::DMA_PER_STAGE * (NSTAGE - 2)>();
+    else
+      wait_vm_le<63>(T::DMA_PER_STAGE * later + E * __builtin_popcount(win));
+    __builtin_amdgcn_s_barrier();
+    if (g + NSTAGE - 1 < total) {
+      const int is = slot == 0 ? NSTAGE - 1 : slot - 1;
+      issue_next(smem + is * T::STAGE_BYTES);
+    }
+    if constexpr (aux_prefetch<EPI, T>())
+      if (ck + 1 == cnk) aux_load<AMODE, EPI, T>(p, cm0, cn0, tid, pre);
+    if (!(p.dbg & 2)) compute(smem + slot * T::STAGE_BYTES);
+    slot = slot == NSTAGE - 1 ? 0 : slot + 1;
+    hist <<= 1;
+    if (++ck == cnk) {
+      bool epi = true;
+      if constexpr (kTail)
+        if (p.tail_r && cu >= p.tail_full) epi = tail_reduce<T>(p, acc, cu - p.tail_full, red, tid);
+      if (epi && !(p.dbg & 1))
+        epilogue<AMODE, EPI, T>(p, acc, cm0, cn0, cu / tiles, red, tid, pre);
+#pragma unroll
+      for (int i = 0; i < FM; ++i)
+#pragma unroll
+        for (int j = 0; j < FN; ++j) acc[i][j] = (f32x4){0.f, 0.f, 0.f, 0.f};
+      hist |= 1u;
+      ck = 0;
+      if (++ci < rounds) {
+        cu = unit_at(ci);
+        unit_geom(cu, cm0, cn0, ckb, cnk);
+      }
+    }
+  }
diff --git a/dfu-multimodal_amd/csrc/gemm_table.h b/dfu-multimodal_amd/csrc/gemm_table.h
--- a/dfu-multimodal_amd/csrc/gemm_table.h
+++ b/dfu-multimodal_amd/csrc/gemm_table.h
@@ -37,6 +37,11 @@
 #undef X
 }
 
+struct dfu_gemm_desc;
+namespace dfu {
+int gemm_group_member_args(const dfu_gemm_desc* d, int split, float* slab, GemmArgs* a);
+}
+
 #define DFU_ENTRY(A, B, E, TMv, TNv, TID)                                             \
   {                                                                                   \
     A, B, E, TID, &dfu::gemm_kernel<A, B, E, TMv, TNv>, dfu::Tile<TMv, TNv>::LDS_BYTES, \
diff --git a/dfu-multimodal_amd/dfu_hip/_lib.py b/dfu-multimodal_amd/dfu_hip/_lib.py
--- a/dfu-multimodal_amd/dfu_hip/_lib.py
+++ b/dfu-multimodal_amd/dfu_hip/_lib.py
@@ -77,6 +77,8 @@
     "dfu_gemm_set_persistent": [I32],
     "dfu_gemm_set_inkernel_reduce": [I32],
     "dfu_gemm_set_tail_split": [I32],
+    "dfu_gemm_group": [ctypes.POINTER(GemmDesc), I32, P, I64, I32, P],
+    "dfu_gemm_group_ws_bytes": [ctypes.POINTER(GemmDesc), I32, I32],
     "dfu_gemm_f32": [I32, I32, I32, P, I64, I64, P, I64, I64, P, I64, P, I32, I32, P, I64, P],
     "dfu_gemm_f32_workspace_bytes": [I32, I32, I32],
     "dfu_pack_conv_weight": [P, P, I32, I32, I32, I32, P],
@@ -165,6 +167,7 @@
     "dfu_binary_eval_counts": [P, P, P, I32, P, P],
 }
 _RESTYPE = {"dfu_last_error_string": c_char_p, "dfu_gemm_workspace_bytes": c_int64,
+            "dfu_gemm_group_ws_bytes": c_int64,
             "dfu_gemm_f32_workspace_bytes": c_int64, "dfu_bn_finalize_ws_bytes": c_int64,
             "dfu_bn_bwd_finalize_ws_bytes": c_int64, "dfu_stem_wgrad_ws_bytes": c_int64,
             "dfu_bn_bwd_ws_bytes": c_int64}
diff --git a/dfu-multimodal_amd/dfu_hip/functional.py b/dfu-multimodal_amd/dfu_hip/functional.py
--- a/dfu-multimodal_amd/dfu_hip/functional.py
+++ b/dfu-multimodal_amd/dfu_hip/functional.py
@@ -454,6 +454,25 @@
         ops.gemm(g.k, N, M, dy_rows, g.k, x_rows, 0, acc, N, a_mode=L.OPND_MNMAJOR,
                  b_mode=L.OPND_CONV_WGRAD_X, epilogue=L.EPI_F32_ACC, conv=g)
         ops.conv_grad_krsc_to_oihw(acc, dw)
+
+
+_RESNET_WGRAD_GROUP = os.environ.get("DFU_RESNET_WGRAD_GROUP", "1") != "0"
+
+
+def conv_wgrad_member(dy_rows, x_rows, geom, dw):
+    g = geom
+    M = g.n * g.p * g.q
+    if g.r == 1 and g.s == 1 and g.stride == 1 and g.pad == 0:
+        return ops.wgrad_member(g.k, g.c, M, dy_rows, g.k, x_rows, g.c, dw, g.c), None
+    N = g.r * g.s * g.c
+    scratch = None
+    if krsc_strided(dw) or (g.r == 1 and g.s == 1):
+        out = _rows2d(dw)
+    else:
+        out = scratch = _empty((g.k, N), F32, dy_rows.device)
+        ops.zero_(scratch)
+    return ops.wgrad_member(g.k, N, M, dy_rows, g.k, x_rows, 0, out, N,
+                            b_mode=L.OPND_CONV_WGRAD_X, conv=g), scratch
 
 
 def _geom(conv, B, H, W):
@@ -685,9 +704,19 @@
         g = rows_view(nhwc_bf16(gout))
         M1, M2 = y1.shape[0], y3.shape[0]
 
+        group, group_w, group_post = [], [], []
+
         def wgrad(conv, dy, x, geom):
             if wants(conv.weight):
-                conv_wgrad(dy, x, geom, grad_buffer(conv.weight))
+                dw = grad_buffer(conv.weight)
+                if _RESNET_WGRAD_GROUP:
+                    m, scratch = conv_wgrad_member(dy, x, geom, dw)
+                    group.append(m)
+                    group_w.append(conv.weight)
+                    if scratch is not None:
+                        group_post.append((scratch, dw))
+                    return
+                conv_wgrad(dy, x, geom, dw)
                 grads_done(conv.weight)
 
         dy3 = torch.empty_like(y3)
@@ -726,6 +755,11 @@
                            w_t=conv1x1_weight_T(mm.get("downsample")[0], gd))
             dx = from_rows(dxr, B, H, W, Cin)
         wgrad(mm["conv1"], dy1, xr, g1)
+        if group:
+            ops.gemm_group(group)
+            for scratch, dw in group_post:
+                ops.conv_grad_krsc_to_oihw(scratch, dw)
+            grads_done(*group_w)
         n_params = len(ctx.needs_input_grad) - 2
         return (dx,) + (None,) * n_params + (None,)
 
diff --git a/dfu-multimodal_amd/dfu_hip/ops.py b/dfu-multimodal_amd/dfu_hip/ops.py
--- a/dfu-multimodal_amd/dfu_hip/ops.py
+++ b/dfu-multimodal_amd/dfu_hip/ops.py
@@ -124,6 +124,66 @@
                             (A, B, C, bias, aux, aux_out, stats, workspace, a_lo), executed))
 
 
+def wgrad_member(M, N, K, A, lda, B, ldb, C, ldc, b_mode=L.OPND_MNMAJOR, conv=None):
+    return (int(M), int(N), int(K), A, int(lda), B, int(ldb), C, int(ldc), int(b_mode), conv)
+
+
+def _wgrad_desc(m):
+    M, N, K, A, lda, B, ldb, C, ldc, b_mode, conv = m
+    for t, name in ((A, "A"), (B, "B"), (C, "C")):
+        if not t.is_cuda:
+            raise ValueError(f"gemm_group: operand {name} must be on the GPU (there is no host path)")
+    d = L.GemmDesc()
+    d.M, d.N, d.K = M, N, K
+    d.a_mode, d.b_mode = L.OPND_MNMAJOR, b_mode
+    d.A, d.lda = A.data_ptr(), lda
+    d.B, d.ldb = B.data_ptr(), ldb
+    d.C, d.ldc = C.data_ptr(), ldc
+    d.epilogue, d.alpha = L.EPI_F32_ACC, 1.0
+    if conv is not None:
+        d.conv_n, d.conv_h, d.conv_w, d.conv_c = conv.n, conv.h, conv.w, conv.c
+        d.conv_k, d.conv_r, d.conv_s = conv.k, conv.r, conv.s
+        d.conv_stride, d.conv_pad, d.conv_p, d.conv_q = conv.stride, conv.pad, conv.p, conv.q
+    return d
+
+
+gemm_group_calls = 0
+
+
+def gemm_group(members, force_split=0, workspace=None):
+    global gemm_group_calls
+    n = len(members)
+    if n == 0:
+        return
+    lb = lib()
+    descs = (L.GemmDesc * n)(*[_wgrad_desc(m) for m in members])
+    need = lb.dfu_gemm_group_ws_bytes(descs, n, int(force_split))
+    if need < 0:
+        check(L.DFU_E_INVALID, "dfu_gemm_group_ws_bytes")
+    if workspace is None and need > 0:
+        workspace = torch.empty(need, dtype=torch.uint8, device=members[0][7].device)
+    nbytes = workspace.numel() * workspace.element_size() if workspace is not None else 0
+    rc = lb.dfu_gemm_group(descs, n, ptr(workspace), nbytes, int(force_split), stream_ptr())
+    if rc:
+        check(rc, "dfu_gemm_group")
+    gemm_group_calls += 1
+    if gemm_record is not None:
+        for m in members:
+            M, N, K, A, _, B, _, C, _, _, conv = m
+            d = _wgrad_desc(m)
+            ref = ctypes.byref(d)
+            ws = None
+            wsn = lb.dfu_gemm_workspace_bytes(ref)
+            if wsn > 0:
+                ws = torch.empty(wsn, dtype=torch.uint8, device=C.device)
+                d.workspace, d.workspace_bytes = ws.data_ptr(), int(wsn)
+                cnt = tile_counters(C.device)
+                d.tile_counters, d.tile_counters_len = cnt.data_ptr(), cnt.numel()
+            flops = 2.0 * M * N * K
+            gemm_record.append((d, flops, _algorithmic_bytes(d, conv),
+                                (A, B, C, None, None, None, None, ws, None), flops))
+
+
 def gemm_set_tail_split(enable):
     return int(lib().dfu_gemm_set_tail_split(int(bool(enable))))
 
diff --git a/include/dfu_hip.h b/include/dfu_hip.h
--- a/include/dfu_hip.h
+++ b/include/dfu_hip.h
@@ -88,6 +88,9 @@
 int dfu_gemm_set_persistent(int32_t mode);
 int dfu_gemm_set_inkernel_reduce(int32_t enable);
 int dfu_gemm_set_tail_split(int32_t enable);
+int dfu_gemm_group(const dfu_gemm_desc* members, int32_t n, void* workspace,
+                   int64_t workspace_bytes, int32_t force_split, void* stream);
+int64_t dfu_gemm_group_ws_bytes(const dfu_gemm_desc* members, int32_t n, int32_t force_split);
 int dfu_gemm_f32(int32_t M, int32_t N, int32_t K, const float* A, int64_t sam, int64_t sak,
                  const float* B, int64_t sbn, int64_t sbk, float* C, int64_t ldc,
                  const float* bias, int32_t relu, int32_t accumulate, void* workspace,
```

Result: no change. 3170, median of 6 (+0.5%).
